# arkworks-rs/pcd

Hardware: AMD Instinct MI355X
Metric: msm_mscalar_mul_per_s (higher is better)
Workload: dtype u32 (11 x 28-bit unsaturated Montgomery limbs, v_mad_u64_u32 with 64-bit column accumulators); 1 GPU; MNT4-298 G1 variable-base MSM, n=1048576 pairs per GPU (2^20 per GPU), proving-key bases and scalars resident in HBM, scalar distribution uniform; curve=MNT4-298, group=G1, log_n=20, window_bits=20, windows=15

## Files before the change

pcd_amd/csrc/capi_internal.h:

```cpp
#pragma once
#include <string.h>

#include <algorithm>
#include <new>

#include "common.h"

namespace pcd {

const int kFieldLimbs[4] = {5, 5, 12, 12};
const int kCurveFq[4] = {0, 1, 2, 3};
const int kCurveFr[4] = {1, 0, 3, 2};
const int kCurveG2Deg[4] = {2, 3, 2, 3};

inline bool valid_curve(int c) { return c >= 0 && c < 4; }
inline bool valid_field(int f) { return f >= 0 && f < 4; }
inline bool valid_group(int g) { return g == 1 || g == 2; }

template <class Fn>
int guarded(Fn&& body) {
  try { return body(); }
  catch (const std::bad_alloc&) { return PCDHIP_E_OOM; }
  catch (...) { return PCDHIP_E_HIP; }
}

inline int fail(pcdhip_ctx* ctx, hipError_t e) {
  if (ctx) { try { ctx->last_hip_error = hipGetErrorString(e); } catch (...) {} }
  if (e == hipErrorOutOfMemory) return PCDHIP_E_OOM;
  if (e == hipErrorNoDevice || e == hipErrorInvalidDevice) return PCDHIP_E_NO_DEVICE;
  if (e == hipErrorInvalidValue) return PCDHIP_E_ARG;
  return PCDHIP_E_HIP;
}
#define TRY(x) do { hipError_t e_ = (x); if (e_ != hipSuccess) return fail(ctx, e_); } while (0)
#define BIND() do { hipError_t e_ = hipSetDevice(ctx->device); if (e_ != hipSuccess) return fail(ctx, e_); } while (0)

enum { AUX_FFT_X = 0, AUX_FFT_TMP, AUX_A, AUX_B, AUX_C, AUX_Z, AUX_CSR_RP, AUX_CSR_COL, AUX_CSR_COEF, AUX_SCAL, AUX_OUT,
       AUX_G16, AUX_Z_CANON, AUX_H_CANON, AUX_MISC, AUX_FB_TABLE, AUX_FB_JAC, AUX_FB_OUT };

struct Dom { uint32_t n, m; int a; };

template <class T> struct FieldTag { typedef T type; };
template <class Fn>
void with_host_field(int field_id, Fn&& fn) {
  switch (field_id) {
    case 0: fn(FieldTag<Fp<F298A, false>>()); break;
    case 1: fn(FieldTag<Fp<F298B, false>>()); break;
    case 2: fn(FieldTag<Fp<F753A, false>>()); break;
    default: fn(FieldTag<Fp<F753B, false>>()); break;
  }
}

typedef hipError_t (*G1ScaleFn)(hipStream_t, const uint32_t*, const uint32_t*, uint32_t, uint32_t, uint32_t*);
G1ScaleFn g1_scale_entry(int curve_id);

hipError_t zero_flagged(hipStream_t st, uint32_t* pts_dev, uint8_t* flags_dev, const uint8_t* flags_host, size_t n, size_t point_bytes);
void shard_range(size_t n, size_t g, size_t parts, size_t* lo, size_t* hi);
int bases_upload_single(pcdhip_ctx* ctx, int curve_id, int group_id, const uint64_t* xy, const uint8_t* inf, size_t n, pcdhip_bases** out);
int msm_common(pcdhip_ctx* ctx, const pcdhip_bases* bases, size_t offset, const uint32_t* scalars_dev, size_t n, uint64_t* out_xyz,
               bool out_on_device = false);
int ensure_side_streams(pcdhip_ctx* ctx);
int drop_side_streams(pcdhip_ctx* ctx, bool partial);
bool pipe_pending(const pcdhip_ctx* ctx);
void drain_peers(pcdhip_ctx* ctx);

int msm_short_common(pcdhip_ctx* ctx, const pcdhip_bases* bases, size_t offset, const uint32_t* scalars_dev, size_t n, uint64_t* out_xyz);
int msm_short_async(pcdhip_ctx* ctx, const pcdhip_bases* bases, size_t offset, const uint32_t* scalars_dev, size_t n, uint32_t* out_dev);
int msm_short_host(pcdhip_ctx* ctx, const pcdhip_bases* bases, size_t offset, const uint64_t* scalars, size_t n, uint64_t* out_xyz);
int msm_short_batch_async(pcdhip_ctx* ctx, const pcdhip_bases* bases, const MsmShortBatchIn* items, size_t k, uint32_t* out_dev,
                          size_t out_stride_words, const uint32_t** err_dev = nullptr, uint32_t* launches = nullptr);

int pick_domain(int field_id, size_t min_size, Dom* d);
int get_tables(pcdhip_ctx* ctx, int field_id, int log_n, const FftTables** out);
int get_mixed_tables(pcdhip_ctx* ctx, int field_id, const Dom& d, const FftTables** out);
int domain_transform(pcdhip_ctx* ctx, int field_id, const Dom& d, uint32_t* v, uint32_t* tmp, int inverse, int coset, float* pass_ms,
                     int* npasses);

size_t csr_bytes(const pcdhip_csr* m, const FieldEntry& fe, size_t off[6]);
int validate_csr(const pcdhip_csr* m, size_t num_cols);
int upload_csr_to(pcdhip_ctx* ctx, const pcdhip_csr* m, const FieldEntry& fe, size_t num_cols, char* d, DevCsr* out);
int upload_csr(pcdhip_ctx* ctx, int slot, const pcdhip_csr* m, const FieldEntry& fe, size_t num_cols, DevCsr* out);
int upload_three(pcdhip_ctx* ctx, const pcdhip_csr* A, const pcdhip_csr* B, const pcdhip_csr* C, const FieldEntry& fe, size_t num_vars,
                 DevCsr out[3]);
int witness_chain_dev(pcdhip_ctx* ctx, int field_id, const DevCsr& mat, int k, const uint32_t* z_dev, size_t num_inputs, const Dom& d, int slot,
                      bool transforms = true);
int witness_finish_dev(pcdhip_ctx* ctx, int field_id, const Dom& d, const uint32_t* b_at = nullptr, const uint32_t* c_at = nullptr);
int witness_map_dev(pcdhip_ctx* ctx, int field_id, const DevCsr mats[3], const uint32_t* z_dev, size_t num_inputs, Dom* dom_out,
                    hipEvent_t after_spmv = nullptr);

struct HostCsrT {
  std::vector<uint64_t> rp;
  std::vector<uint32_t> col;
  std::vector<uint64_t> coeff;
  pcdhip_csr view;
};
int transpose_csr(const pcdhip_csr* m, size_t cols, size_t limbs, HostCsrT* t, const uint32_t* perm = nullptr, size_t rows_out = 0);

void negate_point(int curve_id, int group_id, uint64_t* xy);
void scalar_lincomb(int fr, const uint64_t* const* a, const uint64_t* const* b, size_t n, uint64_t* out);

}

struct pcdhip_pvk {
  int curve_id = 0;
  size_t num_inputs = 0;
  std::vector<uint64_t> alpha, beta, neg_gamma, neg_delta, gamma_abc, alpha_beta , gt_one;
  std::vector<uint8_t> gamma_abc_inf;
  pcdhip_bases* abc = nullptr;
  uint32_t* abc_dev = nullptr;
  size_t abc_tables_off = 0;
};
constexpr size_t PVK_TABLE_INPUTS = 256;
```

pcd_amd/csrc/capi_msm.hip:

```cpp
#include <mutex>

#include "capi_internal.h"

using namespace pcd;

namespace {
__global__ void __launch_bounds__(256) zero_flagged_kernel(uint32_t* __restrict__ pts, const uint8_t* __restrict__ flags, size_t n_words,
                                                            uint32_t words_per_point) {
  const size_t i = (size_t)blockIdx.x * blockDim.x + threadIdx.x;
  if (i < n_words && flags[i / words_per_point]) pts[i] = 0;
}

int lane_reserve_of(const pcdhip_ctx* ctx) {
  int r = ctx->lane_reserve;
  if (r < 0) { const char* e = getenv("PCDHIP_LANE_RESERVE"); r = e ? atoi(e) : 8; }
  return r < 0 ? 0 : r;
}
hipStream_t masked_lane_of(int device, int cus, int reserve, hipError_t* err) {
  static std::mutex mu;
  static std::map<std::pair<int, int>, hipStream_t> pool;
  std::lock_guard<std::mutex> lock(mu);
  auto it = pool.find({device, reserve});
  if (it != pool.end()) { *err = hipSuccess; return it->second; }
  std::vector<uint32_t> mask((cus + 31) / 32, 0u);
  for (int i = 0; i < cus - reserve; i++) mask[i / 32] |= 1u << (i % 32);
  hipStream_t s = nullptr;
  *err = hipExtStreamCreateWithCUMask(&s, (uint32_t)mask.size(), mask.data());
  if (*err == hipSuccess) pool[{device, reserve}] = s;
  return s;
}
int make_side_streams(pcdhip_ctx* ctx) {
  int least = 0, greatest = 0;
  TRY(hipDeviceGetStreamPriorityRange(&least, &greatest));
  const bool lane_mode = ctx->g16_schedule == 2;
  int cus = 0;
  if (hipDeviceGetAttribute(&cus, hipDeviceAttributeMultiprocessorCount, ctx->device) != hipSuccess || cus <= 0) cus = 256;
  const int normal = (least + greatest) / 2;
  for (int k = 0; k < 6; k++) {
    int prio = lane_mode ? (k < 2 ? greatest : k < 4 ? normal : least) : (k < 2 ? greatest : k == 2 ? normal : least);
    static const char* side_prio = getenv("PCDHIP_SIDE_PRIO");
    if (side_prio && !strcmp(side_prio, "low")) prio = least;
    if (side_prio && !strcmp(side_prio, "mid")) prio = k < 3 ? normal : least;
    TRY(hipStreamCreateWithPriority(&ctx->g16_streams[k], hipStreamNonBlocking, prio));
    TRY(hipEventCreate(&ctx->g16_begin[k]));
    TRY(hipEventCreate(&ctx->g16_end[k]));
  }
  if (lane_mode) {
    int reserve = lane_reserve_of(ctx);
    if (reserve >= cus) reserve = 0;
    if (reserve > 0) {
      hipError_t e = hipSuccess;
      ctx->lane.stream = masked_lane_of(ctx->device, cus, reserve, &e);
      TRY(e);
    } else {
      TRY(hipStreamCreateWithPriority(&ctx->lane_stream, hipStreamNonBlocking, least));
      ctx->lane.stream = ctx->lane_stream;
    }
    ctx->lane.cus = cus - reserve;
  }
  TRY(hipEventCreateWithFlags(&ctx->g16_ready, hipEventDisableTiming));
  return PCDHIP_OK;
}
}

namespace pcd {
int msm_coarse_tile_knob() {
  static const int knob = [] {
    const char* e = getenv("PCDHIP_COARSE_TILE");
    if (!e || *e < '0' || *e > '9') return -1;
    const int v = atoi(e);
    return v == 0 || (v >= (int)MSM_STAGE_TILE_MIN && v <= (int)MSM_STAGE_TILE_MAX) ? v : -1;
  }();
  return knob;
}

int msm_bin_stage_knob() {
  static const int knob = [] {
    const char* e = getenv("PCDHIP_BIN_STAGE");
    return e && e[0] == '0' && e[1] == 0 ? 0 : -1;
  }();
  return knob;
}

hipError_t zero_flagged(hipStream_t st, uint32_t* pts_dev, uint8_t* flags_dev, const uint8_t* flags_host, size_t n, size_t point_bytes) {
  if (!flags_host || !n) return hipSuccess;
  hipError_t e = hipMemcpyAsync(flags_dev, flags_host, n, hipMemcpyHostToDevice, st);
  if (e != hipSuccess) return e;
  const size_t nw = n * (point_bytes / 4);
  hipLaunchKernelGGL(zero_flagged_kernel, dim3((unsigned)((nw + 255) / 256)), dim3(256), 0, st, pts_dev, flags_dev, nw, (uint32_t)(point_bytes / 4));
  return hipGetLastError();
}

void shard_range(size_t n, size_t g, size_t parts, size_t* lo, size_t* hi) {
  const size_t base = n / parts, rem = n % parts;
  *lo = g * base + std::min(g, rem);
  *hi = *lo + base + (g < rem ? 1 : 0);
}
int bases_upload_single(pcdhip_ctx* ctx, int curve_id, int group_id, const uint64_t* xy, const uint8_t* inf, size_t n, pcdhip_bases** out) {
  BIND();
  const GroupEntry& ge = group_entry(curve_id, group_id);
  const size_t abi_b = (size_t)ge.point_abi_words * 4, int_b = (size_t)ge.base_stride_words * 4;
  pcdhip_bases* b = new (std::nothrow) pcdhip_bases();
  if (!b) return PCDHIP_E_OOM;
  b->curve_id = curve_id; b->group_id = group_id; b->n = n; b->dptr = nullptr; b->c = 0; b->groups = 1;
  if (ctx->precompute != 0 && n >= 64) {
    const bool full = ctx->precompute < 0;
    const int c = ctx->msm_c ? ctx->msm_c : std::max(6, msm_pick_window(n, ge.scalar_bits, full ? 1 : 0) + ctx->msm_c_bias);
    const int W = msm_num_windows(ge.scalar_bits, c);
    b->c = c;
    b->groups = full ? W : std::min(W, ctx->precompute);
  }
  hipError_t e = hipErrorOutOfMemory;
  while (true) {
    const size_t want = std::max<size_t>(n, 1) * int_b * b->groups;
    e = (ctx->precompute_budget && want > ctx->precompute_budget && b->groups > 1) ? hipErrorOutOfMemory : hipMalloc(&b->dptr, want);
    if (e == hipSuccess || b->groups == 1) break;
    (void)hipGetLastError();
    b->groups = (b->groups + 1) / 2;
  }
  if (e != hipSuccess) { (void)hipGetLastError(); delete b; return fail(ctx, e); }
  if (b->groups == 1) b->c = 0;
  e = ctx->aux_ws.ensure(AUX_MISC, std::max<size_t>(n, 1) * (abi_b + 1) + 64);
  char* stage = (char*)ctx->aux_ws.buf[AUX_MISC];
  if (e == hipSuccess) e = hipMemcpyAsync(stage, xy, n * abi_b, hipMemcpyHostToDevice, ctx->stream);
  if (e == hipSuccess) e = zero_flagged(ctx->stream, (uint32_t*)stage, (uint8_t*)stage + n * abi_b, inf, n, abi_b);
  if (e == hipSuccess) e = ge.points_in(ctx->stream, (const uint32_t*)stage, (uint32_t)n, b->dptr);
  if (e == hipSuccess && b->groups > 1) {
    const int W = msm_num_windows(ge.scalar_bits, b->c);
    const int Wg = (W + b->groups - 1) / b->groups;
    e = ge.precompute(ctx->stream, b->dptr, (uint32_t)n, b->groups, b->c * Wg);
  }
  if (e == hipSuccess && inf) {
    std::vector<uint32_t> bits((n + 31) / 32 + 1, 0u);
    bool any = false;
    for (size_t i = 0; i < n; i++) if (inf[i]) { bits[i >> 5] |= 1u << (i & 31); any = true; }
    if (any) {
      e = hipMalloc((void**)&b->inf_bits, bits.size() * 4);
      if (e == hipSuccess) e = hipMemcpyAsync(b->inf_bits, bits.data(), bits.size() * 4, hipMemcpyHostToDevice, ctx->stream);
      if (e == hipSuccess) e = hipStreamSynchronize(ctx->stream);
    }
  }
  if (e == hipSuccess) e = hipStreamSynchronize(ctx->stream);
  if (e != hipSuccess) { (void)hipFree(b->dptr); (void)hipFree(b->inf_bits); delete b; return fail(ctx, e); }
  *out = b;
  return PCDHIP_OK;
}

int msm_common(pcdhip_ctx* ctx, const pcdhip_bases* bases, size_t offset, const uint32_t* scalars_dev, size_t n,
               uint64_t* out_xyz, bool out_on_device) {
  const GroupEntry& ge = group_entry(bases->curve_id, bases->group_id);
  const size_t jac_b = (size_t)ge.point_words / 2 * 3 * 4, jac_abi_b = (size_t)ge.point_abi_words / 2 * 3 * 4;
  TRY(ctx->msm_ws.ensure(WS_OUT, jac_b + jac_abi_b + 64));
  uint32_t* out_dev = (uint32_t*)ctx->msm_ws.buf[WS_OUT];
  uint32_t* out_abi = out_dev + jac_b / 4;
  TRY(ge.msm(ctx->msm_ws, ctx->stream, bases->view(offset), scalars_dev, (uint32_t)n, out_dev, ctx->msm_c, ctx->msm_chunk,
             ctx->msm_sort, ctx->msm_profile ? &ctx->msm_tm : nullptr, nullptr, MSM_SHARE_NONE));
  if (out_on_device) { TRY(ge.jac_out(ctx->stream, out_dev, 1, (uint32_t*)out_xyz)); return PCDHIP_OK; }
  TRY(ge.jac_out(ctx->stream, out_dev, 1, out_abi));
  TRY(hipMemcpyAsync(out_xyz, out_abi, jac_abi_b, hipMemcpyDeviceToHost, ctx->stream));
  uint32_t too_wide = 0;
  if (ctx->msm_ws.last_err_dev) TRY(hipMemcpyAsync(&too_wide, ctx->msm_ws.last_err_dev, 4, hipMemcpyDeviceToHost, ctx->stream));
  TRY(hipStreamSynchronize(ctx->stream));
  return too_wide ? PCDHIP_E_ARG : PCDHIP_OK;
}

int ensure_side_streams(pcdhip_ctx* ctx) {
  if (ctx->g16_ready) return PCDHIP_OK;
  const int rc = make_side_streams(ctx);
  if (rc) (void)drop_side_streams(ctx, true);
  return rc;
}
int drop_side_streams(pcdhip_ctx* ctx, bool partial) {
  if (!ctx->g16_ready && !partial) return PCDHIP_OK;
  BIND();
  if (!partial) TRY(hipDeviceSynchronize());
  for (int k = 0; k < 6; k++) {
    if (ctx->g16_streams[k]) { (void)hipStreamDestroy(ctx->g16_streams[k]); ctx->g16_streams[k] = nullptr; }
    if (ctx->g16_begin[k]) { (void)hipEventDestroy(ctx->g16_begin[k]); ctx->g16_begin[k] = nullptr; }
    if (ctx->g16_end[k]) { (void)hipEventDestroy(ctx->g16_end[k]); ctx->g16_end[k] = nullptr; }
  }
  if (ctx->lane_stream) { (void)hipStreamDestroy(ctx->lane_stream); ctx->lane_stream = nullptr; }
  ctx->lane = MsmLane();
  if (ctx->g16_ready) (void)hipEventDestroy(ctx->g16_ready);
  ctx->g16_ready = nullptr;
  return PCDHIP_OK;
}
bool pipe_pending(const pcdhip_ctx* ctx) {
  for (int k = 0; k < pcdhip_ctx::PIPE_SLOTS; k++) if (ctx->pipe_busy[k]) return true;
  return false;
}

void drain_peers(pcdhip_ctx* ctx) {
  for (pcdhip_ctx* C : ctx->peers) { if (hipSetDevice(C->device) == hipSuccess) (void)hipStreamSynchronize(C->stream); }
  (void)hipSetDevice(ctx->device);
  (void)hipStreamSynchronize(ctx->stream);
}
}

namespace {
int msm_submit_common(pcdhip_ctx* ctx, const pcdhip_bases* bases, size_t offset, const pcdhip_buf* scalars, size_t scalar_offset, size_t n,
                      uint64_t* out_xyz_device, size_t out_slot_stride, int* ticket) {
  if (!ctx || !bases || !scalars || !ticket || !bases->shards.empty()) return PCDHIP_E_ARG;
  if (offset + n > bases->n || scalar_offset + n > scalars->n || n >= (1ull << 31)) return PCDHIP_E_ARG;
  if (scalars->field_id != kCurveFr[bases->curve_id]) return PCDHIP_E_ARG;
  BIND();
  int rc = ensure_side_streams(ctx);
  if (rc) return rc;
  int slot = -1;
  for (int t = 0; t < pcdhip_ctx::PIPE_SLOTS; t++) {
    const int k = (ctx->pipe_next + t) % pcdhip_ctx::PIPE_SLOTS;
    if (!ctx->pipe_busy[k]) { slot = k; break; }
  }
  if (slot < 0) return PCDHIP_E_ARG;
  ctx->pipe_next = (slot + 1) % pcdhip_ctx::PIPE_SLOTS;
  if (!ctx->pipe_host) TRY(hipHostMalloc((void**)&ctx->pipe_host, pcdhip_ctx::PIPE_SLOTS * pcdhip_ctx::PIPE_HOST_WORDS * 8, hipHostMallocDefault));
  if (!ctx->pipe_done[slot]) TRY(hipEventCreateWithFlags(&ctx->pipe_done[slot], hipEventDisableTiming));
  bool prev_bad = false;
  if (ctx->pipe_partial[slot]) {
    TRY(hipEventSynchronize(ctx->pipe_done[slot]));
    ctx->pipe_partial[slot] = false;
    prev_bad = (uint32_t)ctx->pipe_host[(size_t)slot * pcdhip_ctx::PIPE_HOST_WORDS + pcdhip_ctx::PIPE_HOST_WORDS - 1] != 0;
  }
  const GroupEntry& ge = group_entry(bases->curve_id, bases->group_id);
  const size_t jac_b = (size_t)ge.point_words / 2 * 3 * 4, jac_abi_b = (size_t)ge.point_abi_words / 2 * 3 * 4;
  MsmWorkspace& ws = ctx->g16_ws[2 + slot];
  hipStream_t sk = ctx->g16_streams[2 + slot];
  TRY(ws.ensure(WS_OUT, jac_b + jac_abi_b + 64));
  uint32_t* out_dev = (uint32_t*)ws.buf[WS_OUT];
  uint32_t* out_abi = out_xyz_device ? (uint32_t*)((char*)out_xyz_device + (size_t)slot * out_slot_stride) : out_dev + jac_b / 4;
  TRY(hipEventRecord(ctx->g16_ready, ctx->stream));
  TRY(hipStreamWaitEvent(sk, ctx->g16_ready, 0));
  const size_t sw = (size_t)kFieldLimbs[scalars->field_id] * 2;
  ws.lane = ctx->g16_schedule == 2 && ctx->pipe_lane && ctx->lane.stream ? &ctx->lane : nullptr;
  const hipError_t me = ge.msm(ws, sk, bases->view(offset), scalars->dptr + scalar_offset * sw, (uint32_t)n, out_dev, ctx->msm_c, ctx->msm_chunk, ctx->msm_sort,
                               nullptr, nullptr, MSM_SHARE_NONE);
  ws.lane = nullptr;
  TRY(me);
  TRY(ge.jac_out(sk, out_dev, 1, out_abi));
  uint64_t* host = ctx->pipe_host + (size_t)slot * pcdhip_ctx::PIPE_HOST_WORDS;
  host[pcdhip_ctx::PIPE_HOST_WORDS - 1] = 0;
  if (!out_xyz_device) TRY(hipMemcpyAsync(host, out_abi, jac_abi_b, hipMemcpyDeviceToHost, sk));
  if (ws.last_err_dev) TRY(hipMemcpyAsync(&host[pcdhip_ctx::PIPE_HOST_WORDS - 1], ws.last_err_dev, 4, hipMemcpyDeviceToHost, sk));
  TRY(hipEventRecord(ctx->pipe_done[slot], sk));
  ctx->pipe_busy[slot] = true;
  ctx->pipe_out_bytes[slot] = out_xyz_device ? 0 : jac_abi_b;
  *ticket = slot;
  return prev_bad ? PCDHIP_E_PREV_TICKET : PCDHIP_OK;
}

int msm_sharded_impl(pcdhip_ctx* ctx, const pcdhip_bases* bases, size_t offset, const uint64_t* scalars, size_t n, uint64_t* out_xyz,
                     uint32_t* too_wide) {
  const size_t G = bases->shards.size();
  const GroupEntry& ge = group_entry(bases->curve_id, bases->group_id);
  const size_t jb = (size_t)ge.point_abi_words / 2 * 3 * 4, ji = (size_t)ge.point_words / 2 * 3 * 4;
  const size_t sl = (size_t)kFieldLimbs[kCurveFr[bases->curve_id]];
  BIND();
  TRY(ctx->aux_ws.ensure(AUX_MISC, (G + 1) * jb + 64 * ji + 64));
  uint32_t* d = (uint32_t*)ctx->aux_ws.buf[AUX_MISC];
  uint32_t* gather = d + jb / 4;
  uint32_t* scratch = d + (G + 1) * jb / 4;
  for (size_t g = 0; g < G; g++) {
    const size_t lo = std::max(offset, bases->shard_lo[g]), hi = std::min(offset + n, bases->shard_lo[g + 1]);
    pcdhip_ctx* C = ctx->peers[g];
    if (hi <= lo) {
      TRY(hipSetDevice(ctx->device));
      TRY(hipMemsetAsync((char*)gather + g * jb, 0, jb, ctx->stream));
      continue;
    }
    const pcdhip_bases* sh = bases->shards[g];
    const size_t ng = hi - lo;
    C->msm_sort = ctx->msm_sort;
    {
      pcdhip_ctx* ctx = C;
      BIND();
      const size_t sbytes = ng * sl * 8;
      TRY(C->msm_ws.ensure(WS_SCAL, std::max<size_t>(sbytes, 8)));
      TRY(C->msm_ws.ensure(WS_OUT, ji + jb + 64));
      TRY(hipMemcpyAsync(C->msm_ws.buf[WS_SCAL], scalars + (lo - offset) * sl, sbytes, hipMemcpyHostToDevice, C->stream));
      uint32_t* out_dev = (uint32_t*)C->msm_ws.buf[WS_OUT];
      uint32_t* out_abi = out_dev + ji / 4;
      TRY(ge.msm(C->msm_ws, C->stream, sh->view(lo - bases->shard_lo[g]), (const uint32_t*)C->msm_ws.buf[WS_SCAL], (uint32_t)ng, out_dev, C->msm_c,
                 C->msm_chunk, C->msm_sort, nullptr, nullptr, MSM_SHARE_NONE));
      TRY(ge.jac_out(C->stream, out_dev, 1, out_abi));
      if (C->msm_ws.last_err_dev) TRY(hipMemcpyAsync(&too_wide[g], C->msm_ws.last_err_dev, 4, hipMemcpyDeviceToHost, C->stream));
    }
    const uint32_t* out_abi = (const uint32_t*)C->msm_ws.buf[WS_OUT] + ji / 4;
    TRY(hipSetDevice(C->device));
    TRY(hipMemcpyPeerAsync((char*)gather + g * jb, ctx->device, out_abi, C->device, jb, C->stream));
    if (C != ctx) {
      if (!C->xstream_ev) TRY(hipEventCreateWithFlags(&C->xstream_ev, hipEventDisableTiming));
      TRY(hipEventRecord(C->xstream_ev, C->stream));
      TRY(hipSetDevice(ctx->device));
      TRY(hipStreamWaitEvent(ctx->stream, C->xstream_ev, 0));
    }
  }
  BIND();
  TRY(ge.points_sum(ctx->stream, gather, (uint32_t)G, scratch, d));
  TRY(hipMemcpyAsync(out_xyz, d, jb, hipMemcpyDeviceToHost, ctx->stream));
  for (size_t g = 1; g < G; g++) { TRY(hipSetDevice(ctx->peers[g]->device)); TRY(hipStreamSynchronize(ctx->peers[g]->stream)); }
  BIND();
  TRY(hipStreamSynchronize(ctx->stream));
  for (size_t g = 0; g < G; g++) if (too_wide[g]) return PCDHIP_E_ARG;
  return PCDHIP_OK;
}
int msm_sharded(pcdhip_ctx* ctx, const pcdhip_bases* bases, size_t offset, const uint64_t* scalars, size_t n, uint64_t* out_xyz) {
  if (ctx->peers.size() != bases->shards.size() || ctx->peers.size() > 64) return PCDHIP_E_ARG;
  uint32_t too_wide[64] = {0};
  const int rc = msm_sharded_impl(ctx, bases, offset, scalars, n, out_xyz, too_wide);
  if (rc) drain_peers(ctx);
  return rc;
}

int points_sum_common(pcdhip_ctx* ctx, int curve_id, int group_id, const uint64_t* xyz, size_t n, uint64_t* out_xyz, bool in_on_device) {
  if (!ctx || !valid_curve(curve_id) || !valid_group(group_id) || (!xyz && n) || !out_xyz || (n >> 24)) return PCDHIP_E_ARG;
  BIND();
  const GroupEntry& ge = group_entry(curve_id, group_id);
  const size_t jb = (size_t)ge.point_abi_words / 2 * 3 * 4, ji = (size_t)ge.point_words / 2 * 3 * 4;
  TRY(ctx->aux_ws.ensure(AUX_MISC, (n + 1) * jb + 64 * ji + 64));
  uint32_t* d = (uint32_t*)ctx->aux_ws.buf[AUX_MISC];
  uint32_t* scratch = d + (n + 1) * jb / 4;
  const uint32_t* in = (const uint32_t*)xyz;
  if (!in_on_device) {
    TRY(hipMemcpyAsync(d + jb / 4, xyz, n * jb, hipMemcpyHostToDevice, ctx->stream));
    in = d + jb / 4;
  }
  TRY(ge.points_sum(ctx->stream, in, (uint32_t)n, scratch, d));
  TRY(hipMemcpyAsync(out_xyz, d, jb, hipMemcpyDeviceToHost, ctx->stream));
  TRY(hipStreamSynchronize(ctx->stream));
  return PCDHIP_OK;
}
}

extern "C" {

int pcdhip_bases_upload(pcdhip_ctx* ctx, int curve_id, int group_id, const uint64_t* xy, const uint8_t* inf, size_t n,
                        pcdhip_bases** out) {
  if (!ctx || !out || !valid_curve(curve_id) || !valid_group(group_id) || (!xy && n) || n >= (1ull << 31)) return PCDHIP_E_ARG;
  if (ctx->peers.size() <= 1) return bases_upload_single(ctx, curve_id, group_id, xy, inf, n, out);
  *out = nullptr;
  return guarded([&]() -> int {
    pcdhip_bases* b = new pcdhip_bases();
    b->curve_id = curve_id; b->group_id = group_id; b->n = n; b->dptr = nullptr; b->c = 0; b->groups = 1;
    const size_t G = ctx->peers.size(), pl = (size_t)pcdhip_point_limbs(curve_id, group_id);
    b->shard_lo.resize(G + 1);
    for (size_t g = 0; g < G; g++) {
      size_t lo, hi;
      shard_range(n, g, G, &lo, &hi);
      b->shard_lo[g] = lo; b->shard_lo[g + 1] = hi;
      pcdhip_ctx* C = ctx->peers[g];
      C->precompute = ctx->precompute; C->precompute_budget = ctx->precompute_budget; C->msm_c = ctx->msm_c;
      pcdhip_bases* sh = nullptr;
      int rc = bases_upload_single(C, curve_id, group_id, xy + lo * pl, inf ? inf + lo : nullptr, hi - lo, &sh);
      if (rc) { pcdhip_bases_free(ctx, b); return rc; }
      b->shards.push_back(sh);
    }
    *out = b;
    return PCDHIP_OK;
  });
}
int pcdhip_set_precompute(pcdhip_ctx* ctx, int mode) {
  if (!ctx || mode < -1 || mode == 1) return PCDHIP_E_ARG;
  ctx->precompute = mode;
  return PCDHIP_OK;
}
int pcdhip_set_precompute_budget(pcdhip_ctx* ctx, size_t bytes_per_vector) {
  if (!ctx) return PCDHIP_E_ARG;
  ctx->precompute_budget = bytes_per_vector;
  return PCDHIP_OK;
}
int pcdhip_get_precompute_budget(pcdhip_ctx* ctx, size_t* bytes_per_vector) {
  if (!ctx || !bytes_per_vector) return PCDHIP_E_ARG;
  *bytes_per_vector = ctx->precompute_budget;
  return PCDHIP_OK;
}
void pcdhip_bases_free(pcdhip_ctx* ctx, pcdhip_bases* bases) {
  if (!bases) return;
  for (size_t g = 0; g < bases->shards.size(); g++)
    pcdhip_bases_free(ctx && g < ctx->peers.size() ? ctx->peers[g] : ctx, bases->shards[g]);
  bases->shards.clear();
  if (ctx) (void)hipSetDevice(ctx->device);
  (void)hipFree(bases->dptr);
  (void)hipFree(bases->inf_bits);
  delete bases;
}
int pcdhip_bases_info(const pcdhip_bases* bases, size_t n, int* window_bits, int* windows, int* copies) {
  if (!bases || !window_bits || !windows || !copies) return PCDHIP_E_ARG;
  if (!bases->shards.empty()) return pcdhip_bases_info(bases->shards[0], 0, window_bits, windows, copies);
  const GroupEntry& ge = group_entry(bases->curve_id, bases->group_id);
  const int c = bases->groups > 1 ? bases->c : msm_pick_window(n ? n : bases->n, ge.scalar_bits, 0);
  *window_bits = c;
  *windows = msm_num_windows(ge.scalar_bits, c);
  *copies = bases->groups;
  return PCDHIP_OK;
}
int pcdhip_msm_config(pcdhip_ctx* ctx, int window_bits, int chunk) {
  if (!ctx || window_bits < 0 || window_bits > 24 || chunk < 0) return PCDHIP_E_ARG;
  ctx->msm_c = window_bits;
  ctx->msm_chunk = (uint32_t)chunk;
  return PCDHIP_OK;
}
int pcdhip_msm_set_sort(pcdhip_ctx* ctx, int mode) {
  if (!ctx || mode < 0 || mode > 4) return PCDHIP_E_ARG;
  ctx->msm_sort = (ctx->msm_sort & ~15) | mode;
  return PCDHIP_OK;
}
int pcdhip_msm_set_bin_stage(pcdhip_ctx* ctx, int cap) {
  if (!ctx || cap < -1 || cap > (int)MSM_BIN_STAGE_CAP) return PCDHIP_E_ARG;
  const std::vector<pcdhip_ctx*> one{ctx};
  for (pcdhip_ctx* c : ctx->peers.empty() ? one : ctx->peers) {
    c->msm_ws.bin_stage = cap;
    for (pcd::MsmWorkspace& w : c->g16_ws) w.bin_stage = cap;
  }
  return PCDHIP_OK;
}
int pcdhip_msm_set_accumulate(pcdhip_ctx* ctx, int mode, int chunk, int min_pairs) {
  if (!ctx || mode < 0 || mode > 2 || chunk < 0 || chunk > 1024 || (chunk && chunk < 2) || min_pairs < 0 || min_pairs > 255) return PCDHIP_E_ARG;
  ctx->msm_sort = (ctx->msm_sort & 15) | (mode << 4) | (chunk << 8) | (min_pairs << 20);
  return PCDHIP_OK;
}
int pcdhip_msm_profile(pcdhip_ctx* ctx, int on) {
  if (!ctx) return PCDHIP_E_ARG;
  ctx->msm_profile = on != 0;
  return PCDHIP_OK;
}
int pcdhip_msm_last_plan(pcdhip_ctx* ctx, uint32_t out[2]) {
  if (!ctx || !out) return PCDHIP_E_ARG;
  out[0] = ctx->msm_tm.entries; out[1] = ctx->msm_tm.chunk;
  return PCDHIP_OK;
}
int pcdhip_msm_last_timings(pcdhip_ctx* ctx, float out_ms[8]) {
  if (!ctx || !out_ms) return PCDHIP_E_ARG;
  const MsmTimings& t = ctx->msm_tm;
  float v[8] = {t.digits, t.scan, t.scatter, t.accumulate, t.fixup, t.tail, t.horner, t.total};
  memcpy(out_ms, v, sizeof v);
  return PCDHIP_OK;
}

int pcdhip_msm_ticket_status(pcdhip_ctx* ctx, int slot) {
  if (!ctx || slot < 0 || slot >= pcdhip_ctx::PIPE_SLOTS || ctx->pipe_busy[slot] || !ctx->pipe_partial[slot]) return PCDHIP_E_ARG;
  BIND();
  TRY(hipEventSynchronize(ctx->pipe_done[slot]));
  ctx->pipe_partial[slot] = false;
  return (uint32_t)ctx->pipe_host[(size_t)slot * pcdhip_ctx::PIPE_HOST_WORDS + pcdhip_ctx::PIPE_HOST_WORDS - 1] ? PCDHIP_E_PREV_TICKET : PCDHIP_OK;
}
int pcdhip_msm_submit(pcdhip_ctx* ctx, const pcdhip_bases* bases, size_t offset, const pcdhip_buf* scalars, size_t scalar_offset, size_t n,
                      int* ticket) {
  const int rc = msm_submit_common(ctx, bases, offset, scalars, scalar_offset, n, nullptr, 0, ticket);
  return rc == PCDHIP_E_PREV_TICKET ? PCDHIP_OK : rc;
}
int pcdhip_msm_submit_partial(pcdhip_ctx* ctx, const pcdhip_bases* bases, size_t offset, const pcdhip_buf* scalars, size_t scalar_offset, size_t n,
                              uint64_t* out_xyz_device_slots, size_t slot_stride_bytes, int* ticket) {
  if (!out_xyz_device_slots || (slot_stride_bytes & 7)) return PCDHIP_E_ARG;
  return msm_submit_common(ctx, bases, offset, scalars, scalar_offset, n, out_xyz_device_slots, slot_stride_bytes, ticket);
}
int pcdhip_msm_ticket_wait(pcdhip_ctx* ctx, int ticket, void* other_stream) {
  if (!ctx || ticket < 0 || ticket >= pcdhip_ctx::PIPE_SLOTS || !ctx->pipe_busy[ticket]) return PCDHIP_E_ARG;
  BIND();
  TRY(hipStreamWaitEvent((hipStream_t)other_stream, ctx->pipe_done[ticket], 0));
  ctx->pipe_busy[ticket] = false;
  ctx->pipe_partial[ticket] = true;
  return PCDHIP_OK;
}
int pcdhip_msm_collect(pcdhip_ctx* ctx, int ticket, uint64_t* out_xyz) {
  if (!ctx || ticket < 0 || ticket >= pcdhip_ctx::PIPE_SLOTS || !ctx->pipe_busy[ticket] || !out_xyz) return PCDHIP_E_ARG;
  BIND();
  ctx->pipe_busy[ticket] = false;
  TRY(hipEventSynchronize(ctx->pipe_done[ticket]));
  const uint64_t* host = ctx->pipe_host + (size_t)ticket * pcdhip_ctx::PIPE_HOST_WORDS;
  memcpy(out_xyz, host, ctx->pipe_out_bytes[ticket]);
  return (uint32_t)host[pcdhip_ctx::PIPE_HOST_WORDS - 1] ? PCDHIP_E_ARG : PCDHIP_OK;
}

int pcdhip_msm_dev(pcdhip_ctx* ctx, const pcdhip_bases* bases, size_t offset, const pcdhip_buf* scalars, size_t scalar_offset,
                   size_t n, uint64_t* out_xyz) {
  if (!ctx || !bases || !scalars || !out_xyz) return PCDHIP_E_ARG;
  if (!bases->shards.empty()) return PCDHIP_E_ARG;
  if (offset + n > bases->n || scalar_offset + n > scalars->n || n >= (1ull << 31)) return PCDHIP_E_ARG;
  if (scalars->field_id != kCurveFr[bases->curve_id]) return PCDHIP_E_ARG;
  BIND();
  const size_t sw = (size_t)kFieldLimbs[scalars->field_id] * 2;
  return msm_common(ctx, bases, offset, scalars->dptr + scalar_offset * sw, n, out_xyz);
}

int pcdhip_msm_dev_partial(pcdhip_ctx* ctx, const pcdhip_bases* bases, size_t offset, const pcdhip_buf* scalars, size_t scalar_offset,
                           size_t n, uint64_t* out_xyz_device) {
  if (!ctx || !bases || !scalars || !out_xyz_device || !bases->shards.empty()) return PCDHIP_E_ARG;
  if (offset + n > bases->n || scalar_offset + n > scalars->n || n >= (1ull << 31)) return PCDHIP_E_ARG;
  if (scalars->field_id != kCurveFr[bases->curve_id]) return PCDHIP_E_ARG;
  BIND();
  const size_t sw = (size_t)kFieldLimbs[scalars->field_id] * 2;
  return msm_common(ctx, bases, offset, scalars->dptr + scalar_offset * sw, n, out_xyz_device, true);
}

int pcdhip_msm(pcdhip_ctx* ctx, const pcdhip_bases* bases, size_t offset, const uint64_t* scalars, size_t n, uint64_t* out_xyz) {
  if (!ctx || !bases || (!scalars && n) || !out_xyz) return PCDHIP_E_ARG;
  if (offset + n > bases->n || n >= (1ull << 31)) return PCDHIP_E_ARG;
  if (!bases->shards.empty()) return msm_sharded(ctx, bases, offset, scalars, n, out_xyz);
  BIND();
  const size_t sbytes = n * kFieldLimbs[kCurveFr[bases->curve_id]] * 8;
  TRY(ctx->msm_ws.ensure(WS_SCAL, std::max<size_t>(sbytes, 8)));
  TRY(hipMemcpyAsync(ctx->msm_ws.buf[WS_SCAL], scalars, sbytes, hipMemcpyHostToDevice, ctx->stream));
  return msm_common(ctx, bases, offset, (const uint32_t*)ctx->msm_ws.buf[WS_SCAL], n, out_xyz);
}

int pcdhip_points_sum(pcdhip_ctx* ctx, int curve_id, int group_id, const uint64_t* xyz, size_t n, uint64_t* out_xyz) {
  return points_sum_common(ctx, curve_id, group_id, xyz, n, out_xyz, false);
}
int pcdhip_points_sum_dev(pcdhip_ctx* ctx, int curve_id, int group_id, const uint64_t* xyz_device, size_t n, uint64_t* out_xyz) {
  return points_sum_common(ctx, curve_id, group_id, xyz_device, n, out_xyz, true);
}

int pcdhip_to_affine(pcdhip_ctx* ctx, int curve_id, int group_id, const uint64_t* xyz, size_t n, uint64_t* out_xy, uint8_t* out_inf) {
  if (!ctx || !valid_curve(curve_id) || !valid_group(group_id) || (!xyz && n) || !out_xy) return PCDHIP_E_ARG;
  BIND();
  const GroupEntry& ge = group_entry(curve_id, group_id);
  const size_t ab = (size_t)ge.point_abi_words * 4, jb = ab / 2 * 3;
  TRY(ctx->aux_ws.ensure(AUX_MISC, n * (jb + ab) + 64));
  uint32_t* dj = (uint32_t*)ctx->aux_ws.buf[AUX_MISC];
  uint32_t* da = dj + n * jb / 4;
  TRY(hipMemcpyAsync(dj, xyz, n * jb, hipMemcpyHostToDevice, ctx->stream));
  TRY(ge.to_affine(ctx->stream, dj, (uint32_t)n, da));
  TRY(hipMemcpyAsync(out_xy, da, n * ab, hipMemcpyDeviceToHost, ctx->stream));
  TRY(hipStreamSynchronize(ctx->stream));
  if (out_inf) {
    for (size_t i = 0; i < n; i++) {
      const uint64_t* p = out_xy + i * (ab / 8);
      uint64_t o = 0;
      for (size_t k = 0; k < ab / 8; k++) o |= p[k];
      out_inf[i] = (o == 0) ? 1 : 0;
    }
  }
  return PCDHIP_OK;
}

}
```

pcd_amd/csrc/msm.hip.h:

```cpp
#pragma once
#include <cstdlib>
#include <math.h>

#include <algorithm>
#include <atomic>
#include <type_traits>
#include <vector>

#include "ec.hip.h"

namespace pcd {

template <int K>
struct EventSet {
  hipEvent_t e[K] = {};
  bool live = false;
  hipError_t create() {
    for (int i = 0; i < K; i++) { hipError_t r = hipEventCreate(&e[i]); if (r != hipSuccess) return r; }
    live = true;
    return hipSuccess;
  }
  hipEvent_t operator[](int i) const { return e[i]; }
  ~EventSet() { for (int i = 0; i < K; i++) if (e[i]) (void)hipEventDestroy(e[i]); }
};

struct MsmPlan {
  uint32_t n = 0;
  int c = 0;
  int W = 0;
  uint32_t nkeys = 0;
  uint32_t chunk = 0;
};

PCD_HD constexpr int msm_num_windows(int scalar_bits, int c) { return (scalar_bits + c) / c; }

inline int msm_pick_window(size_t n, int scalar_bits, int full_precompute) {
  double best = 1e300;
  int bc = 8;
  for (int c = 6; c <= 22; c++) {
    int W = msm_num_windows(scalar_bits, c);
    int Wg = full_precompute ? 1 : W;
    double cost = (double)W * (double)n * 11.0 + (double)Wg * (double)(1u << c) * 16.0 * 1.3;
    int top = scalar_bits + 1 - (W - 1) * c;
    cost += (double)n / (double)(1u << (top > 20 ? 20 : top)) * 1400.0;
    if (cost < best) { best = cost; bc = c; }
  }
  return bc;
}

constexpr uint32_t MSM_NEG = 0x80000000u;
PCD_DEV uint32_t msm_signed(uint32_t raw, int c, uint32_t& carry, uint32_t& neg) {
  uint32_t d = raw + carry;
  const bool n = d > (1u << (c - 1));
  carry = n ? 1u : 0u;
  neg = n ? MSM_NEG : 0u;
  return n ? (1u << c) - d : d;
}
template <int NS>
PCD_DEV bool msm_scalar_too_wide(const uint32_t* s, int bits) {
  uint32_t o = 0;
#pragma unroll
  for (int k = 0; k < NS; k++) {
    if (32 * k >= bits) o |= s[k];
    else if (32 * (k + 1) > bits) o |= s[k] >> (bits - 32 * k);
  }
  return o != 0;
}
PCD_DEV bool msm_base_is_inf(const uint32_t* __restrict__ inf_bits, uint32_t idx) { return inf_bits && ((inf_bits[idx >> 5] >> (idx & 31u)) & 1u); }
template <int NS>
PCD_DEV uint32_t msm_digit(const uint32_t* s, int w, int c) {
  int bit = w * c;
  int word = bit >> 5, off = bit & 31;
  uint64_t x = s[word];
  if (word + 1 < NS) x |= (uint64_t)s[word + 1] << 32;
  return (uint32_t)(x >> off) & ((1u << c) - 1u);
}

enum { MODE_HIST = 0, MODE_SCATTER = 1, MODE_BIN = 2 };
template <int NS, int MODE>
__global__ void __launch_bounds__(256) msm_digits_kernel(const uint32_t* __restrict__ scalars, uint32_t n, int c, int W, int Wg,
                                                         uint32_t n_total, uint32_t base_offset, uint32_t nkeys,
                                                         uint32_t* __restrict__ cnt, const uint32_t* __restrict__ off,
                                                         uint32_t* __restrict__ sorted_idx, uint32_t* __restrict__ slots, uint32_t cap,
                                                         uint32_t* __restrict__ ones_idx, uint32_t* __restrict__ flag, int skip_ones,
                                                         int scalar_bits, uint32_t* __restrict__ err, const uint32_t* __restrict__ inf_bits) {
  if (MODE == MODE_SCATTER && flag && *flag == 0) return;
  uint32_t i = blockIdx.x * blockDim.x + threadIdx.x;
  bool live = i < n && !msm_base_is_inf(inf_bits, base_offset + i);
  uint32_t s[NS];
  bool is_one = false;
  if (live || (i < n && MODE != MODE_SCATTER && err)) {
    uint32_t hi = 0;
#pragma unroll
    for (int k = 0; k < NS; k++) { s[k] = scalars[(size_t)i * NS + k]; if (k) hi |= s[k]; }
    is_one = live && (hi == 0 && s[0] == 1);
    if (MODE != MODE_SCATTER && err && msm_scalar_too_wide<NS>(s, scalar_bits)) *err = 1u;
  }
  unsigned long long m = __ballot(live && is_one);
  if (m && !skip_ones) {
    int lane = threadIdx.x & 63;
    int leader = __ffsll((long long)m) - 1;
    uint32_t base = 0;
    if (lane == leader) base = atomicAdd(&cnt[nkeys], (uint32_t)__popcll(m));
    if (MODE != MODE_HIST) {
      base = __shfl(base, leader, 64);
      if (live && is_one) {
        uint32_t rank = (uint32_t)__popcll(m & ((1ull << lane) - 1ull));
        if (MODE == MODE_BIN) ones_idx[base + rank] = base_offset + i;
        else sorted_idx[off[nkeys] + base + rank] = base_offset + i;
      }
    }
  }
  if (!live || is_one) return;
  int g = 0, j = 0;
  uint32_t carry = 0, neg;
  for (int w = 0; w < W; w++) {
    uint32_t d = msm_signed(msm_digit<NS>(s, w, c), c, carry, neg);
    if (d != 0) {
      uint32_t key = ((uint32_t)j << c) | d;
      uint32_t pos = atomicAdd(&cnt[key], 1u);
      uint32_t idx = ((uint32_t)g * n_total + base_offset + i) | neg;
      if (MODE == MODE_SCATTER) sorted_idx[off[key] + pos] = idx;
      if (MODE == MODE_BIN) {
        if (pos < cap) slots[(size_t)key * cap + pos] = idx;
        else *flag = 1u;
      }
    }
    if (++j == Wg) { j = 0; g++; }
  }
}

#ifndef PCD_SORT_UNROLL
#define PCD_SORT_UNROLL 4
#endif
constexpr int MSM_SORT_UNROLL = PCD_SORT_UNROLL;
constexpr int MSM_BIN_SHIFT = 9;
#ifndef PCD_MSM_TILE
#define PCD_MSM_TILE 2048
#endif
constexpr int MSM_TILE = PCD_MSM_TILE;
constexpr uint32_t MSM_MAX_BINS = 8192;

template <int NS, bool WRITE>
__global__ void __launch_bounds__(256) msm_coarse_kernel(const uint32_t* __restrict__ scalars, uint32_t n, int c, int W, int Wg,
                                                         uint32_t n_total, uint32_t base_offset, uint32_t nbins,
                                                         uint32_t* __restrict__ gbin ,
                                                         uint64_t* __restrict__ entries, uint32_t* __restrict__ ones_count,
                                                         uint32_t* __restrict__ ones_idx, int scalar_bits, uint32_t* __restrict__ err,
                                                         const uint32_t* __restrict__ inf_bits) {
  extern __shared__ uint32_t lbin[];
  __shared__ uint32_t s_ones[WRITE ? 1 : MSM_TILE];
  __shared__ uint32_t s_nones, s_ones_base;
  for (uint32_t b = threadIdx.x; b < nbins; b += blockDim.x) lbin[b] = 0;
  if (threadIdx.x == 0) s_nones = 0;
  __syncthreads();
  const uint32_t tile0 = blockIdx.x * MSM_TILE;
  for (uint32_t k = threadIdx.x; k < MSM_TILE; k += blockDim.x) {
    uint32_t i = tile0 + k;
    bool live = i < n && !msm_base_is_inf(inf_bits, base_offset + i);
    uint32_t s[NS];
    bool is_one = false;
    if (live || (i < n && !WRITE)) {
      uint32_t hi = 0;
#pragma unroll
      for (int q = 0; q < NS; q++) { s[q] = scalars[(size_t)i * NS + q]; if (q) hi |= s[q]; }
      is_one = live && (hi == 0 && s[0] == 1);
      if (!WRITE && msm_scalar_too_wide<NS>(s, scalar_bits)) *err = 1u;
    }
    if (!WRITE) {
      unsigned long long m = __ballot(live && is_one);
      if (m) {
        int lane = threadIdx.x & 63;
        int leader = __ffsll((long long)m) - 1;
        uint32_t base = 0;
        if (lane == leader) base = atomicAdd(&s_nones, (uint32_t)__popcll(m));
        base = __shfl(base, leader, 64);
        if (live && is_one) s_ones[base + (uint32_t)__popcll(m & ((1ull << lane) - 1ull))] = base_offset + i;
      }
    }
    if (!live || is_one) continue;
    int j = 0;
    uint32_t carry = 0, neg;
    for (int w = 0; w < W; w++) {
      uint32_t d = msm_signed(msm_digit<NS>(s, w, c), c, carry, neg);
      if (d != 0) atomicAdd(&lbin[((((uint32_t)j << c) | d)) >> MSM_BIN_SHIFT], 1u);
      if (++j == Wg) j = 0;
    }
  }
  __syncthreads();
  for (uint32_t b = threadIdx.x; b < nbins; b += blockDim.x) {
    uint32_t cnt = lbin[b];
    if (cnt) {
      uint32_t base = atomicAdd(&gbin[b], cnt);
      if (WRITE) lbin[b] = base;
    }
  }
  if (!WRITE) {
    if (threadIdx.x == 0) s_ones_base = s_nones ? atomicAdd(ones_count, s_nones) : 0u;
    __syncthreads();
    for (uint32_t k = threadIdx.x; k < s_nones; k += blockDim.x) ones_idx[s_ones_base + k] = s_ones[k];
    return;
  }
  __syncthreads();
  for (uint32_t k = threadIdx.x; k < MSM_TILE; k += blockDim.x) {
    uint32_t i = tile0 + k;
    if (i >= n || msm_base_is_inf(inf_bits, base_offset + i)) continue;
    uint32_t s[NS];
    uint32_t hi = 0;
#pragma unroll
    for (int q = 0; q < NS; q++) { s[q] = scalars[(size_t)i * NS + q]; if (q) hi |= s[q]; }
    if (hi == 0 && s[0] <= 1) continue;
    int g = 0, j = 0;
    uint32_t carry = 0, neg;
    for (int w = 0; w < W; w++) {
      uint32_t d = msm_signed(msm_digit<NS>(s, w, c), c, carry, neg);
      if (d != 0) {
        uint32_t key = ((uint32_t)j << c) | d;
        uint32_t pos = atomicAdd(&lbin[key >> MSM_BIN_SHIFT], 1u);
        entries[pos] = ((uint64_t)key << 32) | (uint64_t)(((uint32_t)g * n_total + base_offset + i) | neg);
      }
      if (++j == Wg) { j = 0; g++; }
    }
  }
}

constexpr int MSM_STAGE_G_BITS = 6, MSM_STAGE_IDX_BITS = 11;
constexpr uint32_t MSM_STAGE_TILE_MAX = 1u << MSM_STAGE_IDX_BITS, MSM_STAGE_TILE_MIN = 256;
constexpr int MSM_STAGE_W_MAX = 1 << MSM_STAGE_G_BITS;
constexpr int MSM_STAGE_SIGN_AT = MSM_BIN_SHIFT, MSM_STAGE_G_AT = MSM_BIN_SHIFT + 1, MSM_STAGE_IDX_AT = MSM_STAGE_G_AT + MSM_STAGE_G_BITS;
static_assert(MSM_STAGE_IDX_AT + MSM_STAGE_IDX_BITS <= 32, "staged word: low key bits, sign, group and tile index in 32 bits");
constexpr size_t MSM_STAGE_LDS_BUDGET = 152u * 1024u;
constexpr uint32_t MSM_STAGE_MIN_RUN = 8;
PCD_HD constexpr size_t msm_stage_lds_bytes(uint32_t tile, int W, uint32_t nbins) { return 4 * ((size_t)tile * (size_t)W + 3 * (size_t)nbins + 4); }
PCD_HD constexpr uint32_t msm_stage_tile(int W, uint32_t nbins) {
  if (W < 1 || W > MSM_STAGE_W_MAX || nbins < 1) return 0;
  for (uint32_t t = MSM_STAGE_TILE_MAX; t >= MSM_STAGE_TILE_MIN; t >>= 1)
    if (msm_stage_lds_bytes(t, W, nbins) <= MSM_STAGE_LDS_BUDGET) return (uint64_t)t * (uint32_t)W >= (uint64_t)MSM_STAGE_MIN_RUN * nbins ? t : 0;
  return 0;
}
int msm_coarse_tile_knob();

constexpr int msm_stage_block(int TILE) { return TILE < 1024 ? TILE : 1024; }
template <int NS, int TILE>
__global__ void __launch_bounds__(msm_stage_block(TILE)) msm_coarse_staged_kernel(const uint32_t* __restrict__ scalars, uint32_t n, int c, int W, int Wg,
                                                                                  uint32_t n_total, uint32_t base_offset, uint32_t nbins,
                                                                                  uint32_t* __restrict__ gbin ,
                                                                                  uint64_t* __restrict__ entries, const uint32_t* __restrict__ inf_bits) {
  constexpr int BLOCK = msm_stage_block(TILE), K = TILE / BLOCK, NW = BLOCK / 64;
  static_assert(TILE >= (int)MSM_STAGE_TILE_MIN && TILE <= (int)MSM_STAGE_TILE_MAX && TILE % BLOCK == 0, "tile");
  extern __shared__ uint32_t lds[];
  uint32_t* cur = lds;
  uint32_t* loff = cur + nbins;
  uint32_t* rdelta = loff + nbins + 1;
  uint32_t* buf = rdelta + nbins;
  __shared__ uint32_t s_wsum[NW];
  const uint32_t t = threadIdx.x, tile0 = blockIdx.x * TILE;
  for (uint32_t b = t; b < nbins; b += BLOCK) cur[b] = 0;
  uint32_t s[K][NS];
  bool live[K];
#pragma unroll
  for (int kk = 0; kk < K; kk++) {
    const uint32_t i = tile0 + t + kk * BLOCK;
    live[kk] = i < n && !msm_base_is_inf(inf_bits, base_offset + i);
    uint32_t hi = 0;
#pragma unroll
    for (int q = 0; q < NS; q++) { s[kk][q] = live[kk] ? scalars[(size_t)i * NS + q] : 0u; if (q) hi |= s[kk][q]; }
    if (hi == 0 && s[kk][0] <= 1) live[kk] = false;
  }
  __syncthreads();
#pragma unroll
  for (int kk = 0; kk < K; kk++) {
    if (!live[kk]) continue;
    int j = 0;
    uint32_t carry = 0, neg;
    for (int w = 0; w < W; w++) {
      uint32_t d = msm_signed(msm_digit<NS>(s[kk], w, c), c, carry, neg);
      if (d != 0) atomicAdd(&cur[((((uint32_t)j << c) | d)) >> MSM_BIN_SHIFT], 1u);
      if (++j == Wg) j = 0;
    }
  }
  __syncthreads();
  const uint32_t per = (nbins + BLOCK - 1) / BLOCK;
  const uint32_t blo = min(nbins, t * per), bhi = min(nbins, blo + per);
  uint32_t acc = 0;
  for (uint32_t b = blo; b < bhi; b++) acc += cur[b];
  const uint32_t lane = t & 63, wv = t >> 6;
  uint32_t incl = acc;
  for (int d = 1; d < 64; d <<= 1) { uint32_t o = __shfl_up(incl, d, 64); if ((int)lane >= d) incl += o; }
  if (lane == 63) s_wsum[wv] = incl;
  __syncthreads();
  uint32_t run = incl - acc;
  for (uint32_t q = 0; q < wv; q++) run += s_wsum[q];
  for (uint32_t b = blo; b < bhi; b++) {
    const uint32_t cnt = cur[b];
    loff[b] = run;
    cur[b] = run;
    if (cnt) rdelta[b] = atomicAdd(&gbin[b], cnt) - run;
    run += cnt;
  }
  if (t == BLOCK - 1) loff[nbins] = run;
  __syncthreads();
#pragma unroll
  for (int kk = 0; kk < K; kk++) {
    if (!live[kk]) continue;
    int g = 0, j = 0;
    uint32_t carry = 0, neg;
    for (int w = 0; w < W; w++) {
      uint32_t d = msm_signed(msm_digit<NS>(s[kk], w, c), c, carry, neg);
      if (d != 0) {
        const uint32_t key = ((uint32_t)j << c) | d;
        const uint32_t q = atomicAdd(&cur[key >> MSM_BIN_SHIFT], 1u);
        buf[q] = (key & ((1u << MSM_BIN_SHIFT) - 1u)) | (neg ? 1u << MSM_STAGE_SIGN_AT : 0u) | ((uint32_t)g << MSM_STAGE_G_AT) |
                 ((t + kk * BLOCK) << MSM_STAGE_IDX_AT);
      }
      if (++j == Wg) { j = 0; g++; }
    }
  }
  __syncthreads();
  const uint32_t total = loff[nbins];
  for (uint32_t q = t; q < total; q += BLOCK) {
    const uint32_t word = buf[q];
    uint32_t lo = 0, hi = nbins;
    while (hi - lo > 1) {
      const uint32_t mid = (lo + hi) >> 1;
      if (loff[mid] <= q) lo = mid; else hi = mid;
    }
    const uint32_t key = (lo << MSM_BIN_SHIFT) | (word & ((1u << MSM_BIN_SHIFT) - 1u));
    const uint32_t g = (word >> MSM_STAGE_G_AT) & ((1u << MSM_STAGE_G_BITS) - 1u);
    const uint32_t neg = (word >> MSM_STAGE_SIGN_AT) & 1u ? MSM_NEG : 0u;
    const uint32_t idx = (g * n_total + base_offset + tile0 + (word >> MSM_STAGE_IDX_AT)) | neg;
    entries[rdelta[lo] + q] = ((uint64_t)key << 32) | (uint64_t)idx;
  }
}
template <int NS, int TILE>
hipError_t msm_coarse_staged_launch(hipStream_t st, uint32_t tiles, size_t lds, const uint32_t* scalars, uint32_t n, int c, int W, int Wg,
                                    uint32_t n_total, uint32_t base_offset, uint32_t nbins, uint32_t* gbin, uint64_t* entries,
                                    const uint32_t* inf_bits) {
  static std::atomic<uint64_t> allowed{0};
  int dev = 0;
  hipError_t e = hipGetDevice(&dev);
  if (e != hipSuccess) return e;
  const uint64_t bit = 1ull << (dev & 63);
  if (!(allowed.load(std::memory_order_relaxed) & bit)) {
    e = hipFuncSetAttribute(reinterpret_cast<const void*>(&msm_coarse_staged_kernel<NS, TILE>), hipFuncAttributeMaxDynamicSharedMemorySize,
                            (int)MSM_STAGE_LDS_BUDGET);
    if (e != hipSuccess) return e;
    allowed.fetch_or(bit, std::memory_order_relaxed);
  }
  hipLaunchKernelGGL((msm_coarse_staged_kernel<NS, TILE>), dim3(tiles), dim3(msm_stage_block(TILE)), lds, st, scalars, n, c, W, Wg, n_total,
                     base_offset, nbins, gbin, entries, inf_bits);
  return hipSuccess;
}

static __global__ void __launch_bounds__(1024) msm_bin_scan_kernel(const uint32_t* __restrict__ bin_cnt, uint32_t nbins,
                                                                   uint32_t* __restrict__ bin_base, uint32_t* __restrict__ cursor,
                                                                   const uint32_t* __restrict__ ones_count, uint32_t* __restrict__ off,
                                                                   uint32_t nkeys) {
  __shared__ uint32_t part[1024];
  const uint32_t per = (nbins + 1023) / 1024;
  const uint32_t lo = threadIdx.x * per, hi = min(nbins, lo + per);
  uint32_t acc = 0;
  for (uint32_t b = lo; b < hi; b++) acc += bin_cnt[b];
  part[threadIdx.x] = acc;
  __syncthreads();
  for (int s = 1; s < 1024; s <<= 1) {
    uint32_t t = ((int)threadIdx.x >= s) ? part[threadIdx.x - s] : 0;
    __syncthreads();
    part[threadIdx.x] += t;
    __syncthreads();
  }
  uint32_t run = part[threadIdx.x] - acc;
  for (uint32_t b = lo; b < hi; b++) { bin_base[b] = run; cursor[b] = run; run += bin_cnt[b]; }
  if (threadIdx.x == 1023) {
    uint32_t M = part[1023];
    bin_base[nbins] = M;
    off[nkeys] = M;
    off[nkeys + 1] = M + *ones_count;
  }
}

template <int BLOCK>
__device__ __forceinline__ void msm_bin_scan_counters(uint32_t* hist, uint32_t* wsum, uint32_t lo, uint32_t hbase, uint32_t* __restrict__ off_b) {
  constexpr int KB = 1 << MSM_BIN_SHIFT, PER = KB / BLOCK;
  static_assert(PER >= 1 && PER * BLOCK == KB && BLOCK % 64 == 0, "counters per lane");
  const uint32_t t = threadIdx.x, lane = t & 63, wv = t >> 6;
  uint32_t c[PER], sum = 0;
#pragma unroll
  for (int k = 0; k < PER; k++) { c[k] = hist[PER * t + k]; sum += c[k]; }
  uint32_t incl = sum;
  for (int d = 1; d < 64; d <<= 1) { uint32_t o = __shfl_up(incl, d, 64); if ((int)lane >= d) incl += o; }
  if (lane == 63) wsum[wv] = incl;
  __syncthreads();
  uint32_t ex = incl - sum;
  for (uint32_t q = 0; q < wv; q++) ex += wsum[q];
#pragma unroll
  for (int k = 0; k < PER; k++) {
    hist[PER * t + k] = hbase + ex;
    off_b[PER * t + k] = lo + ex;
    ex += c[k];
  }
  __syncthreads();
}
template <int BLOCK>
__device__ __forceinline__ void msm_bin_sort_two_read(const uint64_t* __restrict__ entries, uint32_t lo, uint32_t hi, uint32_t* __restrict__ sorted_idx,
                                                      uint32_t* __restrict__ off_b, uint32_t* hist, uint32_t* wsum) {
  constexpr uint32_t KB = 1u << MSM_BIN_SHIFT;
  for (uint32_t k = threadIdx.x; k < KB; k += BLOCK) hist[k] = 0;
  __syncthreads();
  for (uint32_t p0 = lo + threadIdx.x; p0 < hi; p0 += MSM_SORT_UNROLL * BLOCK) {
    uint32_t kk[MSM_SORT_UNROLL];
#pragma unroll
    for (int u = 0; u < MSM_SORT_UNROLL; u++) { uint32_t p = p0 + u * BLOCK; kk[u] = p < hi ? (uint32_t)(entries[p] >> 32) & (KB - 1) : KB; }
#pragma unroll
    for (int u = 0; u < MSM_SORT_UNROLL; u++) if (kk[u] < KB) atomicAdd(&hist[kk[u]], 1u);
  }
  __syncthreads();
  msm_bin_scan_counters<BLOCK>(hist, wsum, lo, lo, off_b);
  for (uint32_t p0 = lo + threadIdx.x; p0 < hi; p0 += MSM_SORT_UNROLL * BLOCK) {
    uint64_t e[MSM_SORT_UNROLL];
    uint32_t pos[MSM_SORT_UNROLL];
#pragma unroll
    for (int u = 0; u < MSM_SORT_UNROLL; u++) { uint32_t p = p0 + u * BLOCK; e[u] = p < hi ? entries[p] : ~0ull; }
#pragma unroll
    for (int u = 0; u < MSM_SORT_UNROLL; u++) if (e[u] != ~0ull) pos[u] = atomicAdd(&hist[(uint32_t)(e[u] >> 32) & (KB - 1)], 1u);
#pragma unroll
    for (int u = 0; u < MSM_SORT_UNROLL; u++) if (e[u] != ~0ull) sorted_idx[pos[u]] = (uint32_t)e[u];
  }
}
static __global__ void __launch_bounds__(256) msm_bin_sort_kernel(const uint64_t* __restrict__ entries, const uint32_t* __restrict__ bin_base,
                                                                  uint32_t* __restrict__ sorted_idx, uint32_t* __restrict__ off) {
  constexpr uint32_t KB = 1u << MSM_BIN_SHIFT;
  __shared__ uint32_t hist[KB];
  __shared__ uint32_t wsum[4];
  const uint32_t b = blockIdx.x;
  msm_bin_sort_two_read<256>(entries, bin_base[b], bin_base[b + 1], sorted_idx, off + (size_t)b * KB, hist, wsum);
}

constexpr int MSM_BIN_STAGE_BLOCK = 512, MSM_BIN_STAGE_PER = 36;
constexpr uint32_t MSM_BIN_STAGE_CAP = MSM_BIN_STAGE_BLOCK * MSM_BIN_STAGE_PER;
PCD_HD constexpr size_t msm_bin_stage_lds_bytes() { return 4 * ((size_t)MSM_BIN_STAGE_CAP + 4 + (1u << MSM_BIN_SHIFT) + MSM_BIN_STAGE_BLOCK / 64); }
static_assert(2 * msm_bin_stage_lds_bytes() <= 160u * 1024u && msm_bin_stage_lds_bytes() <= 78u * 1024u, "two workgroups per CU");
int msm_bin_stage_knob();

static __global__ void __launch_bounds__(MSM_BIN_STAGE_BLOCK, 4) msm_bin_sort_staged_kernel(const uint64_t* __restrict__ entries,
                                                                                             const uint32_t* __restrict__ bin_base,
                                                                                             uint32_t* __restrict__ sorted_idx ,
                                                                                             uint32_t* __restrict__ off, uint32_t cap) {
  constexpr uint32_t KB = 1u << MSM_BIN_SHIFT;
  constexpr int BLOCK = MSM_BIN_STAGE_BLOCK, PER = MSM_BIN_STAGE_PER;
  static_assert(MSM_BIN_STAGE_CAP % 4 == 0 && MSM_BIN_STAGE_CAP < (1u << (32 - MSM_BIN_SHIFT)), "16-byte lines; the rank beside the key");
  extern __shared__ __attribute__((aligned(16))) uint32_t bin_lds[];
  uint32_t* buf = bin_lds;
  uint32_t* hist = buf + MSM_BIN_STAGE_CAP + 4;
  uint32_t* wsum = hist + KB;
  const uint32_t b = blockIdx.x, t = threadIdx.x, lo = bin_base[b], hi = bin_base[b + 1], m = hi - lo;
  uint32_t* off_b = off + (size_t)b * KB;
  if (m > min(cap, MSM_BIN_STAGE_CAP)) { msm_bin_sort_two_read<BLOCK>(entries, lo, hi, sorted_idx, off_b, hist, wsum); return; }
  for (uint32_t k = t; k < KB; k += BLOCK) hist[k] = 0;
  __syncthreads();
  uint64_t e[PER];
#pragma unroll
  for (int u = 0; u < PER; u++) { const uint32_t p = lo + t + u * BLOCK; e[u] = p < hi ? entries[p] : 0ull; }
  uint32_t idx[PER], kr[PER];
#pragma unroll
  for (int u = 0; u < PER; u++) {
    const uint32_t k = (uint32_t)(e[u] >> 32) & (KB - 1);
    idx[u] = (uint32_t)e[u];
    kr[u] = ~0u;
    if (lo + t + u * BLOCK < hi) kr[u] = k | (atomicAdd(&hist[k], 1u) << MSM_BIN_SHIFT);
  }
  __syncthreads();
  const uint32_t sh = lo & 3u;
  msm_bin_scan_counters<BLOCK>(hist, wsum, lo, sh, off_b);
#pragma unroll
  for (int u = 0; u < PER; u++)
    if (kr[u] != ~0u) buf[hist[kr[u] & (KB - 1)] + (kr[u] >> MSM_BIN_SHIFT)] = idx[u];
  __syncthreads();
  const uint32_t end = sh + m;
  uint32_t* dst = sorted_idx + (lo - sh);
  for (uint32_t q = 4 * t; q < end; q += 4 * BLOCK) {
    if (q >= sh && q + 4 <= end) {
      *reinterpret_cast<uint4*>(dst + q) = *reinterpret_cast<const uint4*>(buf + q);
    } else {
#pragma unroll
      for (uint32_t w = 0; w < 4; w++) if (q + w >= sh && q + w < end) dst[q + w] = buf[q + w];
    }
  }
}
static hipError_t msm_bin_sort_launch(hipStream_t st, uint32_t nbins, uint32_t cap, const uint64_t* entries, const uint32_t* bin_base,
                                      uint32_t* sorted_idx, uint32_t* off) {
  if (!cap) {
    hipLaunchKernelGGL(msm_bin_sort_kernel, dim3(nbins), dim3(256), 0, st, entries, bin_base, sorted_idx, off);
    return hipSuccess;
  }
  static std::atomic<uint64_t> allowed{0};
  int dev = 0;
  hipError_t e = hipGetDevice(&dev);
  if (e != hipSuccess) return e;
  const uint64_t bit = 1ull << (dev & 63);
  if (!(allowed.load(std::memory_order_relaxed) & bit)) {
    e = hipFuncSetAttribute(reinterpret_cast<const void*>(&msm_bin_sort_staged_kernel), hipFuncAttributeMaxDynamicSharedMemorySize,
                            (int)msm_bin_stage_lds_bytes());
    if (e != hipSuccess) return e;
    allowed.fetch_or(bit, std::memory_order_relaxed);
  }
  hipLaunchKernelGGL(msm_bin_sort_staged_kernel, dim3(nbins), dim3(MSM_BIN_STAGE_BLOCK), msm_bin_stage_lds_bytes(), st, entries, bin_base,
                     sorted_idx, off, std::min(cap, MSM_BIN_STAGE_CAP));
  return hipSuccess;
}

static __global__ void __launch_bounds__(1024) scan_block_sums(const uint32_t* __restrict__ in, uint32_t n, uint32_t per_block,
                                                         uint32_t* __restrict__ block_sums) {
  __shared__ uint32_t sh[1024];
  uint32_t b = blockIdx.x, lo = b * per_block, hi = min(n, lo + per_block);
  uint32_t acc = 0;
  for (uint32_t i = lo + threadIdx.x; i < hi; i += blockDim.x) acc += in[i];
  sh[threadIdx.x] = acc;
  __syncthreads();
  for (int s = 512; s > 0; s >>= 1) { if ((int)threadIdx.x < s) sh[threadIdx.x] += sh[threadIdx.x + s]; __syncthreads(); }
  if (threadIdx.x == 0) block_sums[b] = sh[0];
}
static __global__ void __launch_bounds__(1024) scan_apply(const uint32_t* __restrict__ in, uint32_t n, uint32_t per_block,
                                                    const uint32_t* __restrict__ block_sums, uint32_t nblocks,
                                                    uint32_t* __restrict__ out ) {
  __shared__ uint32_t sh[1024];
  __shared__ uint32_t carry;
  uint32_t b = blockIdx.x, lo = b * per_block, hi = min(n, lo + per_block);
  if (threadIdx.x == 0) { uint32_t a = 0; for (uint32_t k = 0; k < b; k++) a += block_sums[k]; carry = a; }
  __syncthreads();
  for (uint32_t base = lo; base < hi; base += 1024) {
    uint32_t i = base + threadIdx.x;
    uint32_t v = (i < hi) ? in[i] : 0;
    sh[threadIdx.x] = v;
    __syncthreads();
    for (int s = 1; s < 1024; s <<= 1) {
      uint32_t t = ((int)threadIdx.x >= s) ? sh[threadIdx.x - s] : 0;
      __syncthreads();
      sh[threadIdx.x] += t;
      __syncthreads();
    }
    if (i < hi) out[i] = carry + sh[threadIdx.x] - v;
    __syncthreads();
    if (threadIdx.x == 0) carry += sh[1023];
    __syncthreads();
  }
  if (b == nblocks - 1 && threadIdx.x == 0) out[n] = carry;
}

PCD_HD uint64_t msm_plan_rounds(uint32_t M, uint32_t lanes, uint32_t hi) {
  const uint64_t per_round = (uint64_t)lanes * hi;
  return ((uint64_t)M + per_round - 1) / per_round;
}
PCD_HD uint32_t msm_plan_chunk(uint32_t M, uint32_t lanes, uint32_t lo, uint32_t hi) {
  const uint64_t rounds = msm_plan_rounds(M, lanes, hi);
  const uint32_t chunk = rounds ? (uint32_t)(((uint64_t)M + (uint64_t)lanes * rounds - 1) / ((uint64_t)lanes * rounds)) : lo;
  return chunk < lo ? lo : chunk > hi ? hi : chunk;
}
constexpr uint32_t MSM_CHUNK_MAX = 128;
#ifndef PCD_CHUNK_HI
#define PCD_CHUNK_HI 56
#endif
constexpr uint32_t MSM_CHUNK_HI = PCD_CHUNK_HI;
PCD_HD uint64_t msm_plan_word(uint32_t lanes, uint32_t lo, uint32_t hi) { return (uint64_t)lanes | ((uint64_t)lo << 20) | ((uint64_t)hi << 28); }
PCD_HD uint32_t msm_chunk_of_plan(uint32_t M, uint64_t plan) {
  return msm_plan_chunk(M, (uint32_t)(plan & 0xFFFFFu), (uint32_t)(plan >> 20) & 255u, (uint32_t)(plan >> 28) & 255u);
}
struct MsmChunkRule {
  const uint32_t* chunk_dev;
  uint64_t plan;
  uint32_t chunk;
  PCD_DEV uint32_t eval(const uint32_t* __restrict__ off, uint32_t nkeys) const {
    return chunk_dev ? *chunk_dev : plan ? msm_chunk_of_plan(off[nkeys], plan) : chunk;
  }
};

PCD_DEV uint32_t msm_find_key(const uint32_t* __restrict__ off, uint32_t nkeys, uint32_t p) {
  uint32_t lo = 0, hi = nkeys;
  while (hi - lo > 1) { uint32_t mid = (lo + hi) >> 1; if (off[mid] <= p) lo = mid; else hi = mid; }
  return lo;
}

struct MsmEntrySource {
  const uint32_t* sorted_idx;
  const uint32_t* slots;
  const uint32_t* ones_idx;
  const uint32_t* flag;
  uint32_t cap, ones_key;
};
struct MsmCursor {
  uint32_t key, key_start, key_end;
  uint32_t next_end;
  PCD_DEV void seek(const uint32_t* __restrict__ off, uint32_t nkeys, uint32_t p) {
    key = msm_find_key(off, nkeys, p);
    key_start = off[key];
    key_end = off[key + 1];
    next_end = key + 2 <= nkeys ? off[key + 2] : key_end;
  }
  PCD_DEV void advance_to(const uint32_t* __restrict__ off, uint32_t nkeys, uint32_t p) {
    for (int step = 0; step < 4 && p >= key_end; step++) {
      key++; key_start = key_end; key_end = next_end;
      next_end = key + 2 <= nkeys ? off[key + 2] : key_end;
    }
    if (p >= key_end) seek(off, nkeys, p);
  }
};
PCD_DEV uint32_t msm_entry(const MsmEntrySource& src, bool compact, const MsmCursor& cur, uint32_t p) {
  if (cur.key == src.ones_key) return compact && !src.ones_idx ? src.sorted_idx[p] : src.ones_idx[p - cur.key_start];
  return compact ? src.sorted_idx[p] : src.slots[(size_t)cur.key * src.cap + (p - cur.key_start)];
}

#ifndef PCD_BASE_ALIGN
#define PCD_BASE_ALIGN 1
#endif
template <class G>
struct MsmBaseStride {
  static constexpr int W = Aff<typename G::F>::WORDS;
  static constexpr int value = (PCD_BASE_ALIGN && W == 22) ? 32 : W;
};

template <class G>
struct MsmUseXyzz {
  typedef typename G::F F;
#ifndef PCD_XYZZ_753
#define PCD_XYZZ_753 0
#endif
  static constexpr bool value = F::Base::INLINE_ARITH || F::DEG == 2 || (PCD_XYZZ_753 && F::Base::N > 11);
};
template <class G, bool XYZZ = MsmUseXyzz<G>::value>
struct MsmRunPlain {
  typedef typename G::F F;
  typename EC<G>::AccX a = EC<G>::x_infinity();
  PCD_DEV void add(const Aff<F>& q) { a = EC<G>::madd_x(a, q); }
  PCD_DEV void flush(uint32_t* dst) {
    a.X.store(dst); a.Y.store(dst + F::WORDS); a.ZZ.store(dst + 2 * F::WORDS); a.ZZZ.store(dst + 3 * F::WORDS);
    a = EC<G>::x_infinity();
  }
};
template <class G>
struct MsmRunPlain<G, false> {
  typedef typename G::F F;
  Jac<F> a = Jac<F>::infinity();
  PCD_DEV void add(const Aff<F>& q) { a = EC<G>::madd(a, q); }
  PCD_DEV void flush(uint32_t* dst) { a.store(dst); a = Jac<F>::infinity(); }
};
template <class G>
struct MsmRunLazy {
  typedef typename G::F F;
  typename EC<G>::AccLz a = EC<G>::lz_infinity();
  PCD_DEV void add(const Aff<F>& q) { a = EC<G>::madd_lz(a, q); }
  PCD_DEV void flush(uint32_t* dst) {
    if (a.inf) { F::zero().store(dst + 2 * F::WORDS); return; }
#pragma unroll
    for (int i = 0; i < F::N; i++) dst[i] = (uint32_t)a.X.v[i];
    a.Y.store(dst + F::WORDS);
    a.ZZ.store(dst + 2 * F::WORDS);
    a.ZZZ.store(dst + 3 * F::WORDS);
    a = EC<G>::lz_infinity();
  }
};
#ifndef PCD_ACC_LDS
#define PCD_ACC_LDS 0
#endif
#if defined(__HIP_DEVICE_COMPILE__) || defined(__HIPCC__)
template <class G>
struct MsmRunLazyLds {
  typedef typename G::F F;
  typedef uint32_t V4 __attribute__((ext_vector_type(4)));
  typedef __attribute__((address_space(3))) V4* LdsV4;
  static constexpr int CH = (F::N + 3) / 4;
  struct Store {
    LdsV4 box;
    bool is_inf;
    PCD_DEV bool& inf() { return is_inf; }
    PCD_DEV F ld(int slot) const {
      F r;
#pragma unroll
      for (int k = 0; k < CH; k++) {
        const V4 w = box[(slot * CH + k) * 64 + threadIdx.x];
        r.v[4 * k] = w.x;
        if (4 * k + 1 < F::N) r.v[4 * k + 1] = w.y;
        if (4 * k + 2 < F::N) r.v[4 * k + 2] = w.z;
        if (4 * k + 3 < F::N) r.v[4 * k + 3] = w.w;
      }
      return r;
    }
    PCD_DEV void st(int slot, const F& a) {
#pragma unroll
      for (int k = 0; k < CH; k++) {
        V4 w;
        w.x = a.v[4 * k];
        w.y = 4 * k + 1 < F::N ? a.v[4 * k + 1] : 0u;
        w.z = 4 * k + 2 < F::N ? a.v[4 * k + 2] : 0u;
        w.w = 4 * k + 3 < F::N ? a.v[4 * k + 3] : 0u;
        box[(slot * CH + k) * 64 + threadIdx.x] = w;
      }
    }
  };
  Store s;
  PCD_DEV MsmRunLazyLds() {
    __shared__ V4 accbox[4 * CH * 64];
    s.box = (LdsV4)accbox;
    s.is_inf = true;
  }
  PCD_DEV void add(const Aff<F>& q) { EC<G>::madd_lz_st(s, q); }
  PCD_DEV void flush(uint32_t* dst) {
    if (s.is_inf) { F::zero().store(dst + 2 * F::WORDS); return; }
    s.ld(0).store(dst); s.ld(1).store(dst + F::WORDS); s.ld(2).store(dst + 2 * F::WORDS); s.ld(3).store(dst + 3 * F::WORDS);
    s.is_inf = true;
  }
};
#endif
template <class G, bool XYZZ = MsmUseXyzz<G>::value>
struct MsmStoredPlain {
  typedef typename G::F F;
  static constexpr int WORDS = EC<G>::ACCX_WORDS;
  PCD_DEV static Jac<F> load(const uint32_t* p) {
    typename EC<G>::AccX a = {F::load(p), F::load(p + F::WORDS), F::load(p + 2 * F::WORDS), F::load(p + 3 * F::WORDS)};
    return EC<G>::x_to_jac(a);
  }
  static constexpr bool SEPARATE = true;
};
template <class G>
struct MsmStoredPlain<G, false> {
  typedef typename G::F F;
  static constexpr int WORDS = Jac<F>::WORDS;
  PCD_DEV static Jac<F> load(const uint32_t* p) { return Jac<F>::load(p); }
  static constexpr bool SEPARATE = false;
};
template <class G, bool LAZY = LazyCapable<typename G::F>::value>
struct MsmStored : MsmStoredPlain<G> {};
template <class G>
struct MsmStored<G, true> {
  typedef typename G::F F;
  static constexpr int WORDS = EC<G>::ACC_WORDS;
  PCD_DEV static Jac<F> load(const uint32_t* p) {
    typename EC<G>::AccLz a;
    a.ZZ = F::load(p + 2 * F::WORDS);
    if (a.ZZ.is_zero()) return Jac<F>::infinity();
    a.inf = false;
#pragma unroll
    for (int i = 0; i < F::N; i++) a.X.v[i] = (int32_t)p[i];
    a.Y = F::load(p + F::WORDS);
    a.ZZZ = F::load(p + 3 * F::WORDS);
    return EC<G>::lz_to_jac(a);
  }
  static constexpr bool SEPARATE = true;
};

template <class G>
struct MsmAccWaves {
  typedef typename AccOf<G>::type::F FA;
#ifndef PCD_ACC_WAVES_SPLIT
#define PCD_ACC_WAVES_SPLIT 2
#endif
#ifndef PCD_ACC_WAVES_G1
#define PCD_ACC_WAVES_G1 2
#endif
#ifndef PCD_ACC_WAVES_MB298
#define PCD_ACC_WAVES_MB298 2
#endif
  static constexpr int value = !FA::Base::INLINE_ARITH ? (FA::Base::N <= 11 ? PCD_ACC_WAVES_MB298 : 1)
                             : FA::DEG == 1 ? PCD_ACC_WAVES_G1 : AccOf<G>::LANES > 1 ? PCD_ACC_WAVES_SPLIT : 1;
};

template <class G, bool COMPACT>
__global__ void __launch_bounds__(64, MsmAccWaves<G>::value) msm_accumulate_kernel(const uint32_t* __restrict__ bases, const MsmEntrySource src,
                                                            const uint32_t* __restrict__ off, uint32_t nkeys,
                                                            uint32_t chunk, uint32_t* __restrict__ buckets,
                                                            uint32_t* __restrict__ piece_first, uint32_t* __restrict__ piece_last,
                                                            uint64_t plan ) {
  if (plan) chunk = msm_chunk_of_plan(off[nkeys], plan);
  typedef typename AccOf<G>::type GA;
  typedef typename GA::F F;
  typedef EC<GA> E;
  constexpr int RW = MsmStored<GA>::WORDS;
  constexpr uint32_t LANES = AccOf<G>::LANES, PER_WAVE = 64 / LANES;
  if (threadIdx.x >= PER_WAVE * LANES) return;
  uint32_t t = blockIdx.x * PER_WAVE + threadIdx.x / LANES;
  const uint32_t M = off[nkeys];
  uint64_t start64 = (uint64_t)t * chunk;
  if (start64 >= M) return;
  uint32_t start = (uint32_t)start64, end = (uint32_t)min((uint64_t)M, start64 + chunk);
  if (!COMPACT && src.flag && *src.flag != 0) return;
  if (COMPACT && src.flag && *src.flag == 0) return;
  MsmCursor cur;
  cur.seek(off, nkeys, start);
  bool open_start = cur.key_start < start;
#if PCD_ACC_LDS
  typename std::conditional<LazyCapable<F>::value, MsmRunLazyLds<GA>, MsmRunPlain<GA>>::type acc;
#else
  typename std::conditional<LazyCapable<F>::value, MsmRunLazy<GA>, MsmRunPlain<GA>>::type acc;
#endif
  constexpr bool PREFETCH = F::Base::INLINE_ARITH;
  const uint32_t ones_start = off[src.ones_key];
  auto point_of = [&](uint32_t e) {
    Aff<F> q = Aff<F>::load(bases + (size_t)(e & ~MSM_NEG) * MsmBaseStride<G>::value);
    const F ny = q.y.neg();
    if (e & MSM_NEG) q.y = ny;
    return q;
  };
  if constexpr (COMPACT) {
    auto entry_at = [&](uint32_t pos) { return (src.ones_idx && pos >= ones_start) ? src.ones_idx[pos - ones_start] : src.sorted_idx[pos]; };
    Aff<F> nxt;
    if (PREFETCH) nxt = point_of(entry_at(start));
    for (uint32_t p = start; p < end; p++) {
      if (p >= cur.key_end) {
        if (open_start) { acc.flush(piece_first + (size_t)t * RW); open_start = false; }
        else acc.flush(buckets + (size_t)cur.key * RW);
        cur.advance_to(off, nkeys, p);
      }
      if (PREFETCH) {
        const Aff<F> pt = nxt;
        if (p + 1 < end) nxt = point_of(entry_at(p + 1));
        acc.add(pt);
      } else {
        acc.add(point_of(entry_at(p)));
      }
    }
  } else {
    MsmCursor nxt_cur = cur;
    Aff<F> nxt;
    if (PREFETCH) nxt = point_of(msm_entry(src, false, cur, start));
    for (uint32_t p = start; p < end; p++) {
      if (p >= cur.key_end) {
        if (open_start) { acc.flush(piece_first + (size_t)t * RW); open_start = false; }
        else acc.flush(buckets + (size_t)cur.key * RW);
        cur.advance_to(off, nkeys, p);
      }
      if (PREFETCH) {
        const Aff<F> pt = nxt;
        if (p + 1 < end) {
          nxt_cur.advance_to(off, nkeys, p + 1);
          nxt = point_of(msm_entry(src, false, nxt_cur, p + 1));
        }
        acc.add(pt);
      } else {
        acc.add(point_of(msm_entry(src, false, cur, p)));
      }
    }
  }
  bool open_end = cur.key_end > end;
  if (open_end) acc.flush(piece_last + (size_t)t * RW);
  else if (open_start) acc.flush(piece_first + (size_t)t * RW);
  else acc.flush(buckets + (size_t)cur.key * RW);
}

constexpr uint32_t MSM_TREE_CHUNK_MAX = 640, MSM_TREE_MIN_PAIRS = 12;
constexpr uint32_t MSM_SCR = 0x40000000u;
template <class G>
struct MsmTreeCapable {
  typedef typename AccOf<G>::type::F F;
  static constexpr bool value = F::DEG == 1 && AccOf<G>::LANES == 1 && F::Base::N > 11;
};
struct MsmTreeBufs {
  uint32_t* list;
  uint32_t* pairs;
  uint32_t* prefix;
  uint32_t* pts;
  uint32_t cap;
  uint32_t phases;
  PCD_HD static size_t list_words(uint32_t cap) { return (size_t)4 * cap * 64; }
  PCD_HD static size_t pair_words(uint32_t cap) { return (size_t)3 * (cap / 2 + 1) * 64; }
  PCD_HD static size_t prefix_words(uint32_t cap, int fw) { return (size_t)((fw + 3) / 4 * 4) * (cap / 2 + 1) * 64; }
  PCD_HD static size_t pts_words(uint32_t cap, int fw) { return (size_t)2 * ((fw + 3) / 4 * 4) * (cap + cap / 4 + 8) * 64; }
};
PCD_DEV uint32_t msm_wave_max(uint32_t v) {
#pragma unroll
  for (int m = 32; m >= 1; m >>= 1) v = max(v, (uint32_t)__shfl_xor((int)v, m, 64));
  return v;
}
enum { MSM_PK_ADD = 0, MSM_PK_TAKE_B = 1, MSM_PK_TAKE_A = 2, MSM_PK_INF = 3, MSM_PK_DBL = 4 };

static __global__ void msm_tree_plan_kernel(const uint32_t* __restrict__ off, uint32_t nkeys, uint32_t lanes, uint32_t cap, uint32_t forced,
                                            uint32_t* __restrict__ chunk_out) {
  if (blockIdx.x || threadIdx.x) return;
  const uint64_t M = off[nkeys];
  const uint64_t rounds = (M + (uint64_t)lanes * cap - 1) / ((uint64_t)lanes * cap);
  uint32_t chunk = rounds ? (uint32_t)((M + lanes * rounds - 1) / (lanes * rounds)) : 32u;
  chunk = min(max(chunk, 32u), cap);
  *chunk_out = forced ? forced : chunk;
}
template <class G>
__global__ void __launch_bounds__(64, 1) msm_pair_tree_kernel(const uint32_t* __restrict__ bases, const MsmEntrySource src,
                                                              const uint32_t* __restrict__ off, uint32_t nkeys, const uint32_t* __restrict__ chunk_dev,
                                                              const MsmTreeBufs tb, uint32_t min_pairs, uint32_t* __restrict__ buckets,
                                                              uint32_t* __restrict__ piece_first, uint32_t* __restrict__ piece_last) {
  typedef typename AccOf<G>::type GA;
  typedef typename GA::F F;
  constexpr int RW = MsmStored<GA>::WORDS, FW = F::WORDS;
  const uint32_t lane = threadIdx.x;
  const uint32_t M = off[nkeys];
  const uint32_t chunk = *chunk_dev;
  const uint32_t nwaves = (uint32_t)((((uint64_t)M + chunk - 1) / chunk + 63) / 64);
  const bool compact = !(src.slots && src.flag && *src.flag == 0);
  const uint32_t ones_start = off[src.ones_key];
  uint32_t* const LS = tb.list + (size_t)blockIdx.x * MsmTreeBufs::list_words(tb.cap) + lane;
  uint32_t* const PR = tb.pairs + (size_t)blockIdx.x * MsmTreeBufs::pair_words(tb.cap) + lane;
  constexpr int ECH = (FW + 3) / 4, EW = 4 * ECH;
  uint32_t* const PX = tb.prefix + (size_t)blockIdx.x * MsmTreeBufs::prefix_words(tb.cap, FW) + lane * 4;
  uint32_t* const PT = tb.pts + (size_t)blockIdx.x * MsmTreeBufs::pts_words(tb.cap, FW) + lane * 4;
  typedef uint32_t V4 __attribute__((ext_vector_type(4)));
  auto fld_ld = [&](const uint32_t* p) { F r;
#pragma unroll
    for (int c = 0; c < ECH; c++) {
      const V4 v = *reinterpret_cast<const V4*>(p + (size_t)c * 256);
      r.v[4 * c] = v.x;
      if (4 * c + 1 < FW) r.v[4 * c + 1] = v.y;
      if (4 * c + 2 < FW) r.v[4 * c + 2] = v.z;
      if (4 * c + 3 < FW) r.v[4 * c + 3] = v.w;
    }
    return r; };
  auto fld_st = [&](uint32_t* p, const F& a) {
#pragma unroll
    for (int c = 0; c < ECH; c++) {
      V4 v;
      v.x = a.v[4 * c];
      v.y = 4 * c + 1 < FW ? a.v[4 * c + 1] : 0u;
      v.z = 4 * c + 2 < FW ? a.v[4 * c + 2] : 0u;
      v.w = 4 * c + 3 < FW ? a.v[4 * c + 3] : 0u;
      *reinterpret_cast<V4*>(p + (size_t)c * 256) = v;
    } };
  auto x_of = [&](uint32_t loc) {
    const bool scr = (loc & MSM_SCR) != 0;
    if (!__any(scr)) return F::load(bases + (size_t)(loc & ~MSM_NEG) * MsmBaseStride<G>::value);
    if (__all(scr)) return fld_ld(PT + (size_t)(loc & ~MSM_SCR) * (2 * EW * 64));
    F r = F::zero();
    if (scr) r = fld_ld(PT + (size_t)(loc & ~MSM_SCR) * (2 * EW * 64));
    else r = F::load(bases + (size_t)(loc & ~MSM_NEG) * MsmBaseStride<G>::value);
    return r; };
  auto base_point = [&](uint32_t loc) {
    Aff<F> q = Aff<F>::load(bases + (size_t)(loc & ~MSM_NEG) * MsmBaseStride<G>::value);
    const F ny = q.y.neg();
    if (loc & MSM_NEG) q.y = ny;
    return q; };
  auto scratch_point = [&](uint32_t loc) {
    const uint32_t* p = PT + (size_t)(loc & ~MSM_SCR) * (2 * EW * 64);
    Aff<F> q;
    q.x = fld_ld(p); q.y = fld_ld(p + (size_t)EW * 64);
    return q; };
  auto point_of = [&](uint32_t loc) {
    const bool scr = (loc & MSM_SCR) != 0;
    if (!__any(scr)) return base_point(loc);
    if (__all(scr)) return scratch_point(loc);
    Aff<F> q = {F::zero(), F::zero()};
    if (scr) q = scratch_point(loc);
    else q = base_point(loc);
    return q; };
  for (uint32_t w = blockIdx.x; w < nwaves; w += gridDim.x) {
    const uint32_t t = w * 64 + lane;
    const uint64_t start64 = (uint64_t)t * chunk;
    const uint32_t start = start64 < M ? (uint32_t)start64 : M;
    const uint32_t n0 = min(M - start, chunk), end = start + n0;
    uint32_t key_first = 0;
    bool open_start = false;
    if (n0) {
      MsmCursor cur;
      cur.seek(off, nkeys, start);
      key_first = cur.key;
      open_start = cur.key_start < start;
      for (uint32_t i = 0; i < n0; i++) {
        const uint32_t p = start + i;
        if (p >= cur.key_end) cur.advance_to(off, nkeys, p);
        uint32_t e;
        if (compact) e = (src.ones_idx && p >= ones_start) ? src.ones_idx[p - ones_start] : src.sorted_idx[p];
        else e = msm_entry(src, false, cur, p);
        LS[(size_t)(2 * i) * 64] = cur.key;
        LS[(size_t)(2 * i + 1) * 64] = e;
      }
    }
    uint32_t cnt = n0, which = 0, slot_base = 0;
    for (;;) {
      uint32_t* const in = LS + (size_t)which * (2 * tb.cap * 64);
      uint32_t* const out = LS + (size_t)(which ^ 1) * (2 * tb.cap * 64);
      uint32_t np = 0, j = 0;
      for (uint32_t i = 0; i < cnt; j++) {
        const uint32_t k0 = in[(size_t)(2 * i) * 64], l0 = in[(size_t)(2 * i + 1) * 64];
        if (i + 1 < cnt && in[(size_t)(2 * i + 2) * 64] == k0) {
          PR[(size_t)(3 * np) * 64] = l0;
          PR[(size_t)(3 * np + 1) * 64] = in[(size_t)(2 * i + 3) * 64];
          out[(size_t)(2 * j) * 64] = k0;
          out[(size_t)(2 * j + 1) * 64] = MSM_SCR | (slot_base + np);
          np++; i += 2;
        } else {
          out[(size_t)(2 * j) * 64] = k0;
          out[(size_t)(2 * j + 1) * 64] = l0;
          i++;
        }
      }
      const uint32_t np_max = msm_wave_max(np);
      if (np_max < min_pairs) break;
      F run = F::one();
      {
        uint32_t la = 0, lb = 0, la1 = 0, lb1 = 0;
        if (0 < np) { la = PR[0]; lb = PR[(size_t)64]; }
        if (1 < np) { la1 = PR[(size_t)3 * 64]; lb1 = PR[(size_t)4 * 64]; }
        F x1n = F::zero(), x2n = F::zero();
        if (0 < np) { x1n = x_of(la); x2n = x_of(lb); }
        for (uint32_t k = 0; k < np_max; k++) {
          const F x1 = x1n, x2 = x2n;
          const uint32_t ca = la, cb = lb;
          la = la1; lb = lb1;
          if (k + 2 < np) { la1 = PR[(size_t)(3 * k + 6) * 64]; lb1 = PR[(size_t)(3 * k + 7) * 64]; }
          if (k + 1 < np) { x1n = x_of(la); x2n = x_of(lb); }
          F dd = F::one();
          if (k < np) {
            uint32_t kind = MSM_PK_ADD;
            dd = x2 - x1;
            if (__builtin_expect(x1.is_raw_zero() || x2.is_raw_zero() || dd.is_zero(), 0)) {
              const Aff<F> a = point_of(ca), b = point_of(cb);
              if (a.is_inf()) { kind = MSM_PK_TAKE_B; dd = F::one(); }
              else if (b.is_inf()) { kind = MSM_PK_TAKE_A; dd = F::one(); }
              else if (dd.is_zero()) {
                if ((a.y + b.y).is_zero()) { kind = MSM_PK_INF; dd = F::one(); }
                else { kind = MSM_PK_DBL; dd = a.y.dbl(); }
              }
            }
            PR[(size_t)(3 * k + 2) * 64] = kind;
            fld_st(PX + (size_t)k * (EW * 64), run);
          }
          run = F::mul_impl(run, dd);
        }
      }
      F inv = run.inv_gcd();
      {
        Aff<F> an = {F::zero(), F::zero()}, bn = an;
        F pren = F::one();
        uint32_t kindn = MSM_PK_INF, la = 0, lb = 0;
        if (np_max - 1 < np) {
          const uint32_t k = np_max - 1;
          an = point_of(PR[(size_t)(3 * k) * 64]); bn = point_of(PR[(size_t)(3 * k + 1) * 64]);
          kindn = PR[(size_t)(3 * k + 2) * 64];
          pren = fld_ld(PX + (size_t)k * (EW * 64));
        }
        if (np_max >= 2 && np_max - 2 < np) { la = PR[(size_t)(3 * (np_max - 2)) * 64]; lb = PR[(size_t)(3 * (np_max - 2) + 1) * 64]; }
        for (uint32_t k = np_max; k-- > 0;) {
          const bool live = k < np;
          const uint32_t kind = live ? kindn : (uint32_t)MSM_PK_ADD;
          const F ax = an.x, ay = an.y, pre = pren;
          const F sx = an.x + bn.x;
          F dd = F::one(), num = F::zero();
          if (live && kind == MSM_PK_ADD) { dd = bn.x - an.x; num = bn.y - an.y; }
          if (__builtin_expect(__any(kind == MSM_PK_DBL), 0)) {
            if (kind == MSM_PK_DBL) { const F xx = ax.sqr(); dd = ay.dbl(); num = xx.dbl() + xx + GA::mul_by_a(F::one()); }
          }
          F t0 = F::zero(), lam = F::zero();
#pragma nounroll
          for (uint32_t ph = 0; ph < tb.phases; ph++) {
            F u, v;
            if (ph == 0) { u = inv; v = pre; }
            else if (ph == 1) { u = inv; v = dd; }
            else { u = num; v = t0; }
            const F m = F::mul_impl(u, v);
            if (ph == 0) t0 = m;
            else if (ph == 1) inv = m;
            else lam = m;
          }
          if (k >= 1 && k - 1 < np) {
            an = point_of(la); bn = point_of(lb);
            kindn = PR[(size_t)(3 * (k - 1) + 2) * 64];
            pren = fld_ld(PX + (size_t)(k - 1) * (EW * 64));
          }
          if (k >= 2 && k - 2 < np) { la = PR[(size_t)(3 * (k - 2)) * 64]; lb = PR[(size_t)(3 * (k - 2) + 1) * 64]; }
          Aff<F> r;
          r.x = F::sqr_impl(lam) - sx;
          r.y = F::mul_impl(lam, ax - r.x) - ay;
          if (__builtin_expect(__any(live && kind != MSM_PK_ADD && kind != MSM_PK_DBL), 0)) {
            if (live && kind == MSM_PK_TAKE_A) r = point_of(PR[(size_t)(3 * k) * 64]);
            if (live && kind == MSM_PK_TAKE_B) r = point_of(PR[(size_t)(3 * k + 1) * 64]);
            if (live && kind == MSM_PK_INF) r = {F::zero(), F::zero()};
          }
          if (live) {
            uint32_t* p = PT + (size_t)(slot_base + k) * (2 * EW * 64);
            fld_st(p, r.x); fld_st(p + (size_t)EW * 64, r.y);
          }
        }
      }
      slot_base += np_max;
      cnt = j;
      which ^= 1;
    }
    if (n0) {
      const uint32_t* const in = LS + (size_t)which * (2 * tb.cap * 64);
      MsmRunPlain<GA> acc;
      uint32_t key = key_first;
      for (uint32_t i = 0; i < cnt; i++) {
        const uint32_t k0 = in[(size_t)(2 * i) * 64], l0 = in[(size_t)(2 * i + 1) * 64];
        if (k0 != key) {
          if (open_start) { acc.flush(piece_first + (size_t)t * RW); open_start = false; }
          else acc.flush(buckets + (size_t)key * RW);
          key = k0;
        }
        acc.add(point_of(l0));
      }
      const bool open_end = off[key + 1] > end;
      if (open_end) acc.flush(piece_last + (size_t)t * RW);
      else if (open_start) acc.flush(piece_first + (size_t)t * RW);
      else acc.flush(buckets + (size_t)key * RW);
    }
  }
}

template <class G>
struct MsmItems {
  typedef typename SplitOfTail<G>::type GA;
  static constexpr uint32_t LANES = SplitOfTail<G>::LANES, PER_WAVE = 64 / LANES;
  PCD_DEV static bool idle() { return threadIdx.x >= PER_WAVE * LANES; }
  PCD_DEV static uint32_t local() { return threadIdx.x / LANES; }
  PCD_DEV static uint32_t item() { return blockIdx.x * PER_WAVE + threadIdx.x / LANES; }
  static uint32_t grid(uint32_t items) { return (items + PER_WAVE - 1) / PER_WAVE; }
};

static __global__ void __launch_bounds__(256) msm_zero_kernel(uint32_t* __restrict__ cnt, uint32_t n_cnt, uint32_t* __restrict__ ctl4) {
  const uint32_t i = blockIdx.x * blockDim.x + threadIdx.x;
  if (i < n_cnt) cnt[i] = 0;
  if (i < 4) ctl4[i] = 0;
}

#ifndef PCD_SINGLE_ITEM_PLAIN
#define PCD_SINGLE_ITEM_PLAIN 0
#endif
template <class G> struct MsmSingleItem {
  typedef typename std::conditional<PCD_SINGLE_ITEM_PLAIN != 0, typename SplitOf<G>::type, typename SplitOfTail<G>::type>::type GA;
  static constexpr int LANES = PCD_SINGLE_ITEM_PLAIN != 0 ? SplitOf<G>::LANES : SplitOfTail<G>::LANES;
};
template <class G>
__global__ void __launch_bounds__(64) msm_merge_ones_kernel(uint32_t* __restrict__ buckets, uint32_t ones_key) {
  typedef typename MsmSingleItem<G>::GA GA;
  typedef typename GA::F F;
  if (blockIdx.x != 0 || threadIdx.x >= MsmSingleItem<G>::LANES) return;
  Jac<F> a = Jac<F>::load(buckets + (size_t)1 * Jac<F>::WORDS);
  Jac<F> b = Jac<F>::load(buckets + (size_t)ones_key * Jac<F>::WORDS);
  EC<GA>::add(a, b).store(buckets + (size_t)1 * Jac<F>::WORDS);
}

template <class G>
__global__ void __launch_bounds__(64) msm_fixup_kernel(const uint32_t* __restrict__ off, uint32_t nkeys, const MsmChunkRule rule,
                                                       const uint32_t* __restrict__ piece_first, const uint32_t* __restrict__ piece_last,
                                                       const uint32_t* __restrict__ acc_buckets ,
                                                       uint32_t* __restrict__ buckets, uint32_t big_limit, uint32_t* __restrict__ big_count,
                                                       uint32_t* __restrict__ big_list , uint32_t big_cap,
                                                       uint32_t* __restrict__ seg_list , uint32_t seg_len) {
  const uint32_t chunk = rule.eval(off, nkeys);
  typedef typename MsmItems<G>::GA GA;
  typedef typename GA::F F;
  typedef EC<GA> E;
  constexpr int RW = MsmStored<GA>::WORDS;
  if (MsmItems<G>::idle()) return;
  const bool lead = threadIdx.x % MsmItems<G>::LANES == 0;
  const uint32_t item = MsmItems<G>::item();
  if (item < 2) {
    const uint32_t key = item == 0 ? 1u : nkeys - 1;
    const uint32_t lo = off[key], hi = off[key + 1];
    if (hi == lo) F::zero().store(buckets + (size_t)key * Jac<F>::WORDS + 2 * F::WORDS);
    else if (MsmStored<GA>::SEPARATE && hi - (lo / chunk) * chunk <= chunk)
      MsmStored<GA>::load(acc_buckets + (size_t)key * RW).store(buckets + (size_t)key * Jac<F>::WORDS);
    return;
  }
  const uint32_t t0 = item - 2;
  const uint64_t edge = ((uint64_t)t0 + 1) * chunk;
  if (edge >= off[nkeys]) return;
  const uint32_t key = msm_find_key(off, nkeys, (uint32_t)edge - 1);
  const uint32_t lo = off[key], hi = off[key + 1];
  if (hi <= (uint32_t)edge || lo / chunk != t0) return;
  const uint32_t t1 = (hi - 1) / chunk;
  if (t1 - t0 + 1 > big_limit) {
    if (!lead) return;
    uint32_t nseg = (t1 - t0 + seg_len) / seg_len;
    uint32_t slot = atomicAdd(&big_count[0], 1u);
    uint32_t s0 = atomicAdd(&big_count[1], nseg);
    if (slot < big_cap) { big_list[3 * slot] = key; big_list[3 * slot + 1] = s0; big_list[3 * slot + 2] = nseg; }
    for (uint32_t i = 0; i < nseg; i++) {
      uint32_t lo = t0 + i * seg_len, hi = min(t1, lo + seg_len - 1);
      seg_list[3 * (s0 + i)] = lo; seg_list[3 * (s0 + i) + 1] = hi; seg_list[3 * (s0 + i) + 2] = t1;
    }
    return;
  }
  Jac<F> acc = MsmStored<GA>::load(piece_last + (size_t)t0 * RW);
  for (uint32_t u = t0 + 1; u < t1; u++) acc = E::add(acc, MsmStored<GA>::load(piece_last + (size_t)u * RW));
  acc = E::add(acc, MsmStored<GA>::load(piece_first + (size_t)t1 * RW));
  acc.store(buckets + (size_t)key * Jac<F>::WORDS);
}

template <class G, bool ENABLE = true, bool Q = true>
struct MsmPairItems {
  static constexpr bool TWO = ENABLE && TwoLaneOps<G>::value && (MsmItems<G>::LANES == 1 || HalfLanes<typename MsmItems<G>::GA::F>::L == (int)MsmItems<G>::LANES);
  static constexpr bool QUAD = Q && TWO && MsmItems<G>::LANES == 1 && PCD_EC4 != 0;
  static constexpr uint32_t BASE = MsmItems<G>::LANES, LANES = QUAD ? 4 : TWO ? 2 * BASE : BASE, PER_WAVE = 64 / LANES;
  PCD_DEV static bool idle() { return threadIdx.x >= PER_WAVE * LANES; }
  PCD_DEV static uint32_t item() { return blockIdx.x * PER_WAVE + threadIdx.x / LANES; }
  PCD_DEV static uint32_t local() { return threadIdx.x / LANES; }
  PCD_DEV static bool writer() { return QUAD ? (threadIdx.x & 3u) == 0 : (!TWO || (((threadIdx.x & 63u) / BASE) & 1u) == 0); }
  static uint32_t grid(uint32_t items) { return (items + PER_WAVE - 1) / PER_WAVE; }
};
template <class G, bool TWO = MsmPairItems<G, true>::TWO, bool Q = true>
struct MsmPairOps {
  typedef typename MsmItems<G>::GA GA;
  typedef Jac<typename GA::F> J;
  PCD_DEV static J add(const J& a, const J& b) { return EC<GA>::add(a, b); }
  PCD_DEV static J dbl(const J& a) { return EC<GA>::dbl(a); }
};
template <class G, bool Q>
struct MsmPairOps<G, true, Q> {
  typedef typename SplitOfTail<G>::type GA;
  typedef Jac<typename GA::F> J;
  PCD_DEV static J add(const J& a, const J& b) { if constexpr (MsmPairItems<G, true, Q>::QUAD) return EC4<GA>::add4(a, b); else return EC2<GA>::add2(a, b); }
  PCD_DEV static J dbl(const J& a) { if constexpr (MsmPairItems<G, true, Q>::QUAD) return EC4<GA>::dbl4(a); else return EC2<GA>::dbl2(a); }
};
template <class G>
PCD_DEV void msm_wave_tree(Jac<typename MsmPairOps<G>::GA::F> acc, uint32_t* my , uint32_t* dst) {
  typedef MsmPairItems<G> IT;
  typedef MsmPairOps<G> O;
  typedef typename O::GA::F F;
  constexpr uint32_t PW = IT::PER_WAVE;
  const uint32_t it = IT::local();
  const bool live = !IT::idle();
  if (live && IT::writer()) acc.store(my + (size_t)it * Jac<F>::WORDS);
  __syncthreads();
  for (uint32_t s = 32; s > 0; s >>= 1) {
    if (live && it < s && it + s < PW) {
      Jac<F> o = Jac<F>::load(my + (size_t)(it + s) * Jac<F>::WORDS);
      acc = O::add(acc, o);
      if (IT::writer()) acc.store(my + (size_t)it * Jac<F>::WORDS);
    }
    __syncthreads();
  }
  if (live && it == 0 && IT::writer()) acc.store(dst);
  __syncthreads();
}
template <class G>
__global__ void __launch_bounds__(64) msm_big_segments_kernel(const uint32_t* __restrict__ seg_list, const uint32_t* __restrict__ big_count,
                                                              const uint32_t* __restrict__ piece_first, const uint32_t* __restrict__ piece_last,
                                                              uint32_t* __restrict__ partial, uint32_t* __restrict__ scratch) {
  typedef MsmPairItems<G> IT;
  typedef MsmPairOps<G> O;
  typedef typename O::GA GA;
  typedef typename GA::F F;
  constexpr uint32_t PW = IT::PER_WAVE;
  const uint32_t nseg = big_count[1];
  uint32_t* my = scratch + (size_t)blockIdx.x * 64 * Jac<F>::WORDS;
  for (uint32_t sg = blockIdx.x; sg < nseg; sg += gridDim.x) {
    uint32_t lo = seg_list[3 * sg], hi = seg_list[3 * sg + 1], tlast = seg_list[3 * sg + 2];
    Jac<F> acc = Jac<F>::infinity();
    if (!IT::idle())
      for (uint32_t u = lo + IT::local(); u <= hi; u += PW) {
        const uint32_t* src = (u == tlast) ? piece_first : piece_last;
        acc = O::add(acc, MsmStored<GA>::load(src + (size_t)u * MsmStored<GA>::WORDS));
      }
    msm_wave_tree<G>(acc, my, partial + (size_t)sg * Jac<F>::WORDS);
  }
}
template <class G>
__global__ void __launch_bounds__(64) msm_big_bucket_kernel(const uint32_t* __restrict__ big_list, const uint32_t* __restrict__ big_count,
                                                            const uint32_t* __restrict__ partial, uint32_t* __restrict__ buckets,
                                                            uint32_t* __restrict__ scratch) {
  typedef MsmPairItems<G> IT;
  typedef MsmPairOps<G> O;
  typedef typename O::GA GA;
  typedef typename GA::F F;
  constexpr uint32_t PW = IT::PER_WAVE;
  const uint32_t nbig = big_count[0];
  uint32_t* my = scratch + (size_t)blockIdx.x * 64 * Jac<F>::WORDS;
  for (uint32_t b = blockIdx.x; b < nbig; b += gridDim.x) {
    uint32_t key = big_list[3 * b], s0 = big_list[3 * b + 1], ns = big_list[3 * b + 2];
    Jac<F> acc = Jac<F>::infinity();
    if (!IT::idle())
      for (uint32_t u = IT::local(); u < ns; u += PW) acc = O::add(acc, Jac<F>::load(partial + (size_t)(s0 + u) * Jac<F>::WORDS));
    msm_wave_tree<G>(acc, my, buckets + (size_t)key * Jac<F>::WORDS);
  }
}

struct MsmBucketSrc {
  const uint32_t* off;
  const uint32_t* acc_buckets;
  const uint32_t* buckets;
  uint32_t nkeys;
  MsmChunkRule rule;
};
template <class GA>
PCD_DEV Jac<typename GA::F> msm_bucket_at(const MsmBucketSrc& bs, uint32_t chunk, uint32_t key) {
  typedef typename GA::F F;
  if (key != 1) {
    const uint32_t lo = bs.off[key], hi = bs.off[key + 1];
    if (hi == lo) return Jac<F>::infinity();
    if (hi - (lo / chunk) * chunk <= chunk)
      return MsmStored<GA>::load(bs.acc_buckets + (size_t)key * MsmStored<GA>::WORDS);
  }
  return Jac<F>::load(bs.buckets + (size_t)key * Jac<F>::WORDS);
}
template <class G, bool WIDE>
__global__ void __launch_bounds__(64) msm_tail_level_kernel(const MsmBucketSrc bs, uint32_t mA, size_t strideA_in,
                                                            const uint32_t* __restrict__ C_in, uint32_t mC, size_t strideC_in,
                                                            uint32_t* __restrict__ A_out, size_t strideA_out,
                                                            uint32_t* __restrict__ C_out, size_t strideC_out, int k) {
  typedef MsmPairItems<G, WIDE> IT;
  typedef MsmPairOps<G, IT::TWO> O;
  typedef typename O::GA GA;
  typedef typename GA::F F;
  constexpr int PW = Jac<F>::WORDS;
  if (IT::idle()) return;
  uint32_t K = 1u << k;
  uint32_t JA = (mA + K - 1) >> k, JC = (mC + K - 1) >> k;
  uint32_t tid = IT::item();
  uint32_t w = blockIdx.y;
  if (tid < JA) {
    const uint32_t chunk = bs.rule.eval(bs.off, bs.nkeys);
    const uint32_t key1 = w * (uint32_t)strideA_in + 1;
    Jac<F> run = Jac<F>::infinity(), acc = Jac<F>::infinity();
    for (int tt = (int)K - 1; tt >= 0; tt--) {
      uint32_t i = tid * K + tt;
      if (i < mA) run = O::add(run, msm_bucket_at<GA>(bs, chunk, key1 + i));
      acc = O::add(acc, run);
    }
    if (IT::writer()) acc.store(C_out + (w * strideC_out + JC + tid) * PW);
    if (tid >= 1) {
      for (int d = 0; d < k; d++) run = O::dbl(run);
      if (IT::writer()) run.store(A_out + (w * strideA_out + tid - 1) * PW);
    }
  } else if (tid < JA + JC) {
    uint32_t j = tid - JA;
    const uint32_t* Cw = C_in + w * strideC_in * PW;
    Jac<F> acc = Jac<F>::infinity();
    for (uint32_t tt = 0; tt < K; tt++) {
      uint32_t i = j * K + tt;
      if (i < mC) acc = O::add(acc, Jac<F>::load(Cw + (size_t)i * PW));
    }
    if (IT::writer()) acc.store(C_out + (w * strideC_out + j) * PW);
  }
}

template <class G, bool Q = true, bool FIRST = false>
PCD_DEV void msm_tail_pair_item(int role, uint32_t j, uint32_t w, const uint32_t* A_in, uint32_t mA, size_t strideA_in, const uint32_t* C_in,
                                uint32_t mC, size_t strideC_in, uint32_t* A_out, size_t strideA_out, uint32_t* C_out, size_t strideC_out,
                                const MsmBucketSrc* bs = nullptr) {
  typedef MsmPairOps<G, MsmPairItems<G, true>::TWO, Q> O;
  typedef typename O::GA GA;
  typedef typename GA::F F;
  typedef MsmPairItems<G, true, Q> IT;
  constexpr int PW = Jac<F>::WORDS;
  const uint32_t JA = (mA + 1) >> 1, JC = (mC + 1) >> 1;
  if (role < 2) {
    if (j >= JA) return;
    uint32_t chunk = 0;
    if constexpr (FIRST) chunk = bs->rule.eval(bs->off, bs->nkeys);
    auto a_at = [&](uint32_t i) {
      if constexpr (FIRST) return msm_bucket_at<GA>(*bs, chunk, w * (uint32_t)strideA_in + 1 + i);
      else return Jac<F>::load(A_in + (w * strideA_in + i) * PW);
    };
    const bool two = 2 * j + 1 < mA;
    const Jac<F> a0 = a_at(2 * j);
    if (role == 0) {
      if (j == 0) return;
      Jac<F> run = two ? O::add(a0, a_at(2 * j + 1)) : a0;
      run = O::dbl(run);
      if (IT::writer()) run.store(A_out + (w * strideA_out + j - 1) * PW);
    } else {
      Jac<F> acc = two ? O::add(O::dbl(a_at(2 * j + 1)), a0) : a0;
      if (IT::writer()) acc.store(C_out + (w * strideC_out + JC + j) * PW);
    }
  } else {
    if (j >= JC) return;
    const uint32_t* Cw = C_in + w * strideC_in * PW;
    Jac<F> acc = Jac<F>::load(Cw + (size_t)(2 * j) * PW);
    if (2 * j + 1 < mC) acc = O::add(acc, Jac<F>::load(Cw + (size_t)(2 * j + 1) * PW));
    if (IT::writer()) acc.store(C_out + (w * strideC_out + j) * PW);
  }
}
template <class G, bool Q = true>
__global__ void __launch_bounds__(64) msm_tail_pair_kernel(const uint32_t* __restrict__ A_in, uint32_t mA, size_t strideA_in,
                                                           const uint32_t* __restrict__ C_in, uint32_t mC, size_t strideC_in,
                                                           uint32_t* __restrict__ A_out, size_t strideA_out,
                                                           uint32_t* __restrict__ C_out, size_t strideC_out) {
  typedef MsmPairItems<G, true, Q> IT;
  if (IT::idle()) return;
  msm_tail_pair_item<G, Q>((int)blockIdx.z, IT::item(), blockIdx.y, A_in, mA, strideA_in, C_in, mC, strideC_in, A_out, strideA_out, C_out, strideC_out);
}
template <class G, bool Q = true>
__global__ void __launch_bounds__(64) msm_tail_pair_first_kernel(const MsmBucketSrc bs, uint32_t mA, size_t strideA_in,
                                                                 uint32_t* __restrict__ A_out, size_t strideA_out,
                                                                 uint32_t* __restrict__ C_out, size_t strideC_out) {
  typedef MsmPairItems<G, true, Q> IT;
  if (IT::idle()) return;
  msm_tail_pair_item<G, Q, true>((int)blockIdx.z, IT::item(), blockIdx.y, nullptr, mA, strideA_in, nullptr, 0u, 0, A_out, strideA_out, C_out, strideC_out, &bs);
}
constexpr uint32_t MSM_FUSED_WAVES = 4;
#ifndef PCD_QUAD_MAX_ITEMS
#define PCD_QUAD_MAX_ITEMS 4096
#endif
constexpr uint32_t MSM_QUAD_MAX_ITEMS = PCD_QUAD_MAX_ITEMS;
template <class G>
struct MsmFusedTail {
  static constexpr bool ENABLED = !MsmPairOps<G>::GA::F::Base::MAILBOX;
  static uint32_t waves(uint32_t items) { return (items + MsmPairItems<G>::PER_WAVE - 1) / MsmPairItems<G>::PER_WAVE; }
  static bool fits(uint32_t mA, uint32_t mC) { return ENABLED && 2 * waves((mA + 1) >> 1) + waves((mC + 1) >> 1) <= MSM_FUSED_WAVES; }
};
template <class G>
__global__ void __launch_bounds__(64 * MSM_FUSED_WAVES) msm_tail_fused_kernel(const uint32_t* A_in, uint32_t mA, size_t strideA_in, const uint32_t* C_in,
                                                                              uint32_t mC, size_t strideC_in, uint32_t* A0, uint32_t* A1, uint32_t* C0,
                                                                              uint32_t* C1, size_t strideAC, int flip) {
  typedef MsmPairItems<G> IT;
  const uint32_t wave = threadIdx.x >> 6, lane = threadIdx.x & 63u;
  const bool idle = lane >= IT::PER_WAVE * IT::LANES;
  const uint32_t w = blockIdx.x;
  while (mA > 0 || mC > 1) {
    const uint32_t JA = (mA + 1) >> 1, JC = (mC + 1) >> 1;
    uint32_t* A_out = flip ? A1 : A0;
    uint32_t* C_out = flip ? C1 : C0;
    const uint32_t wa = (JA + IT::PER_WAVE - 1) / IT::PER_WAVE;
    const int role = wave < wa ? 0 : wave < 2 * wa ? 1 : 2;
    const uint32_t j = (wave - (uint32_t)role * wa) * IT::PER_WAVE + lane / IT::LANES;
    if (!idle) msm_tail_pair_item<G>(role, j, w, A_in, mA, strideA_in, C_in, mC, strideC_in, A_out, strideAC, C_out, strideAC);
    __syncthreads();
    mA = JA ? JA - 1 : 0;
    mC = JC + JA;
    A_in = A_out; strideA_in = strideAC;
    C_in = C_out; strideC_in = strideAC;
    flip ^= 1;
  }
}

template <class G>
__global__ void __launch_bounds__(64) msm_horner_kernel(const uint32_t* __restrict__ C, size_t strideC, int W, int c, uint32_t* __restrict__ out) {
  typedef typename MsmSingleItem<G>::GA GA;
  typedef typename GA::F F;
  typedef EC<GA> E;
  constexpr int PW = Jac<F>::WORDS;
  if (blockIdx.x != 0 || threadIdx.x >= MsmSingleItem<G>::LANES) return;
  Jac<F> total = Jac<F>::load(C + (size_t)(W - 1) * strideC * PW);
  for (int w = W - 2; w >= 0; w--) {
    for (int d = 0; d < c; d++) total = E::dbl(total);
    total = E::add(total, Jac<F>::load(C + (size_t)w * strideC * PW));
  }
  total.store(out);
}

template <class G>
__global__ void __launch_bounds__(64) points_abi_to_internal_kernel(const uint32_t* __restrict__ abi, uint32_t n, uint32_t* __restrict__ out) {
  typedef typename G::F F;
  uint32_t i = blockIdx.x * blockDim.x + threadIdx.x;
  if (i >= n) return;
  Aff<F>::from_abi(abi + (size_t)i * Aff<F>::ABI_WORDS).store(out + (size_t)i * MsmBaseStride<G>::value);
}
template <class G>
__global__ void __launch_bounds__(64) jac_internal_to_abi_kernel(const uint32_t* __restrict__ in, uint32_t n, uint32_t* __restrict__ abi) {
  typedef typename G::F F;
  uint32_t i = blockIdx.x * blockDim.x + threadIdx.x;
  if (i >= n) return;
  Jac<F> p = Jac<F>::load(in + (size_t)i * Jac<F>::WORDS);
  if (p.is_inf()) p = Jac<F>::infinity();
  p.to_abi(abi + (size_t)i * Jac<F>::ABI_WORDS);
}

template <class G>
__global__ void __launch_bounds__(64) msm_precompute_kernel(uint32_t* __restrict__ pts, uint32_t n, int groups, int shift) {
  typedef typename std::conditional<AccOf<G>::LANES == 1, typename AccOf<G>::type, G>::type GP;
  typedef typename GP::F F;
  typedef EC<GP> E;
  constexpr int BLK = (F::Base::N > 11 || F::DEG > 1) ? 4 : 8;
  uint32_t i = blockIdx.x * blockDim.x + threadIdx.x;
  if (i >= n) return;
  constexpr int STRIDE = MsmBaseStride<G>::value;
  Aff<F> p = Aff<F>::load(pts + (size_t)i * STRIDE);
  if (p.is_inf()) {
    for (int g = 1; g < groups; g++) p.store(pts + ((size_t)g * n + i) * STRIDE);
    return;
  }
  Jac<F> q = {p.x, p.y, F::one()};
  for (int g0 = 1; g0 < groups; g0 += BLK) {
    const int nb = min(BLK, groups - g0);
    F zs[BLK], pre[BLK];
    unsigned infm = 0;
#pragma unroll
    for (int j = 0; j < BLK; j++) {
      if (j < nb) {
        for (int d = 0; d < shift; d++) q = E::dbl(q);
        uint32_t* dst = pts + ((size_t)(g0 + j) * n + i) * STRIDE;
        q.X.store(dst);
        q.Y.store(dst + F::WORDS);
        const bool inf = q.is_inf();
        if (inf) infm |= 1u << j;
        zs[j] = inf ? F::one() : q.Z;
        pre[j] = j ? pre[j - 1] * zs[j] : zs[j];
      }
    }
    F inv = pre[0];
#pragma unroll
    for (int j = 1; j < BLK; j++) if (j == nb - 1) inv = pre[j];
    inv = inv.inv();
    Aff<F> last = {F::zero(), F::zero()};
#pragma unroll
    for (int j = BLK - 1; j >= 0; j--) {
      if (j < nb) {
        const F zi = j ? inv * pre[j - 1] : inv;
        inv = inv * zs[j];
        uint32_t* dst = pts + ((size_t)(g0 + j) * n + i) * STRIDE;
        const F zi2 = zi.sqr();
        Aff<F> a = {F::load(dst) * zi2, F::load(dst + F::WORDS) * zi2 * zi};
        if (infm & (1u << j)) a = {F::zero(), F::zero()};
        a.store(dst);
        if (j == nb - 1) last = a;
      }
    }
    q = (infm >> (nb - 1)) & 1u ? Jac<F>::infinity() : Jac<F>{last.x, last.y, F::one()};
  }
}
template <class G>
hipError_t msm_precompute(hipStream_t st, uint32_t* pts, uint32_t n, int groups, int shift) {
  if (n == 0 || groups <= 1) return hipSuccess;
  hipLaunchKernelGGL((msm_precompute_kernel<G>), dim3((n + 63) / 64), dim3(64), 0, st, pts, n, groups, shift);
  return hipGetLastError();
}

struct MsmLane {
  hipStream_t stream = nullptr;
  int cus = 0;
};

struct MsmWorkspace {
  void* buf[28] = {nullptr};
  size_t cap[28] = {0};
  const MsmLane* lane = nullptr;
  hipEvent_t lane_in = nullptr, lane_out = nullptr;
  const uint32_t* last_err_dev = nullptr;
  int cus = 0;
  int bin_stage = -1;
  hipError_t ensure(int slot, size_t bytes) {
    if (cap[slot] >= bytes) return hipSuccess;
    if (buf[slot]) { hipError_t e = hipFree(buf[slot]); if (e != hipSuccess) return e; buf[slot] = nullptr; cap[slot] = 0; }
    size_t want = bytes + bytes / 8 + 256;
    hipError_t e = hipMalloc(&buf[slot], want);
    if (e != hipSuccess) return e;
    cap[slot] = want;
    return hipSuccess;
  }
  void release() {
    for (int i = 0; i < 28; i++) if (buf[i]) { (void)hipFree(buf[i]); buf[i] = nullptr; cap[i] = 0; }
    if (lane_in) { (void)hipEventDestroy(lane_in); lane_in = nullptr; }
    if (lane_out) { (void)hipEventDestroy(lane_out); lane_out = nullptr; }
  }
};

struct MsmTimings {
  float digits = 0, scan = 0, scatter = 0, accumulate = 0, fixup = 0, tail = 0, horner = 0, total = 0;
  uint32_t entries = 0, chunk = 0;
};

enum { WS_CNT = 0, WS_OFF, WS_BSUM, WS_SORTED, WS_BUCKETS, WS_PFIRST, WS_PLAST, WS_BIG, WS_BIGSCR, WS_A0, WS_A1, WS_C0, WS_C1, WS_OUT, WS_SCAL,
       WS_BIGPART, WS_ONES, WS_SLOTS, WS_CUR, WS_ENTRIES, WS_ACCB, WS_TLIST, WS_TPAIR, WS_TPREFIX, WS_TPTS };

#define PCD_HIP_TRY(x) do { hipError_t e_ = (x); if (e_ != hipSuccess) return e_; } while (0)

struct MsmBasesView {
  const uint32_t* dptr;
  uint32_t n_total;
  uint32_t offset;
  int c;
  int groups;
  const uint32_t* inf_bits = nullptr;
};

struct MsmSharedSort {
  bool valid = false;
  uint32_t n = 0, n_total = 0, offset = 0, tkeys = 0;
  int c = 0, W = 0, groups = 0;
  const uint32_t* scalars = nullptr;
  const uint32_t* inf_bits = nullptr;
  MsmEntrySource src{};
  const uint32_t* off = nullptr;
  hipEvent_t ready = nullptr;
};
enum { MSM_SHARE_NONE = 0, MSM_SHARE_PRODUCE = 1, MSM_SHARE_CONSUME = 2 };

template <class G>
hipError_t msm_run(MsmWorkspace& ws, hipStream_t st, const MsmBasesView& bv, const uint32_t* scalars_dev, uint32_t n,
                   uint32_t* out_dev, int c_override, uint32_t chunk_override, int sort_mode, MsmTimings* tm,
                   MsmSharedSort* share = nullptr, int share_role = MSM_SHARE_NONE) {
  const int acc_mode = (sort_mode >> 4) & 3;
  const uint32_t tree_chunk = ((uint32_t)sort_mode >> 8) & 0xFFFu, tree_min_pairs = ((uint32_t)sort_mode >> 20) & 0xFFu;
  sort_mode &= 15;
  const bool single_pass = sort_mode == 1;
  const uint32_t* bases_dev = bv.dptr;
  typedef typename G::F F;
  constexpr int NS = G::FR::N32;
  constexpr int PW = Jac<F>::WORDS;
  constexpr size_t PB = (size_t)PW * 4;
  if (n == 0) { ws.last_err_dev = nullptr; Jac<F> inf = Jac<F>::infinity(); return hipMemcpyAsync(out_dev, &inf, PB, hipMemcpyHostToDevice, st); }
  MsmPlan pl;
  pl.n = n;
  pl.c = bv.groups > 1 ? bv.c : (c_override ? c_override : msm_pick_window(n, G::FR::BITS, 0));
  pl.W = msm_num_windows(G::FR::BITS, pl.c);
  const int Wg = (pl.W + bv.groups - 1) / bv.groups;
  pl.nkeys = (uint32_t)Wg << pl.c;
  const uint64_t maxM = (uint64_t)n * pl.W;
  pl.chunk = chunk_override ? chunk_override : 40;
  int& cus = ws.cus;
  if (!cus) {
    int dev = 0;
    if (hipGetDevice(&dev) != hipSuccess || hipDeviceGetAttribute(&cus, hipDeviceAttributeMultiprocessorCount, dev) != hipSuccess || cus <= 0) cus = 256;
  }
  bool use_tree = false;
  uint32_t tree_cap = 0;
  const uint32_t* tree_chunk_dev = nullptr;
  if constexpr (MsmTreeCapable<G>::value) {
    use_tree = acc_mode == 2 && (uint64_t)bv.n_total * bv.groups < MSM_SCR;
    if (use_tree) {
      tree_cap = tree_chunk ? tree_chunk : MSM_TREE_CHUNK_MAX;
      pl.chunk = tree_cap;
    }
  }
  const MsmLane* lane = ws.lane;
  const int plan_cus = lane && lane->cus > 0 ? lane->cus : cus;
  uint32_t acc_lanes = 0, chunk_lo = 0;
  static const uint32_t chunk_hi_env = getenv("PCDHIP_CHUNK_HI") ? (uint32_t)atoi(getenv("PCDHIP_CHUNK_HI")) : 0u;
  const uint32_t chunk_hi = chunk_hi_env >= 16 && chunk_hi_env <= MSM_CHUNK_MAX ? chunk_hi_env : MSM_CHUNK_HI;
  if (!chunk_override && !use_tree) {
    acc_lanes = (uint32_t)plan_cus * 4 * MsmAccWaves<G>::value * (64 / AccOf<G>::LANES);
    chunk_lo = (uint32_t)std::min<uint64_t>(40, std::max<uint64_t>(16, (maxM + 4ull * acc_lanes - 1) / (4ull * acc_lanes)));
    pl.chunk = chunk_lo;
  }
  const uint64_t plan_word = acc_lanes && acc_lanes < (1u << 20) ? msm_plan_word(acc_lanes, chunk_lo, chunk_hi) : 0u;
  if (acc_lanes && !plan_word) pl.chunk = 40;
  if (maxM >= 0xFFFFFFF0ull || (uint64_t)bv.n_total * bv.groups >= 0x7FFFFFF0ull) return hipErrorInvalidValue;

  EventSet<9> ev;
  if (tm) PCD_HIP_TRY(ev.create());
  auto mark = [&](int i) -> hipError_t { return tm ? hipEventRecord(ev[i], st) : hipSuccess; };

  const uint32_t tkeys = pl.nkeys + 1, ones_key = pl.nkeys;
  const bool consume = share && share_role == MSM_SHARE_CONSUME && share->valid && share->n == n && share->n_total == bv.n_total &&
                       share->offset == bv.offset && share->tkeys == tkeys && share->c == pl.c && share->W == pl.W &&
                       share->groups == bv.groups && share->scalars == scalars_dev &&
                       (share->inf_bits == nullptr || share->inf_bits == bv.inf_bits);
  PCD_HIP_TRY(ws.ensure(WS_CNT, (size_t)tkeys * 4 + 16));
  PCD_HIP_TRY(ws.ensure(WS_OFF, ((size_t)tkeys + 1) * 4));
  const uint32_t scan_per_block = 16384;
  const uint32_t scan_blocks = (tkeys + scan_per_block - 1) / scan_per_block;
  PCD_HIP_TRY(ws.ensure(WS_BSUM, (size_t)scan_blocks * 4));
  PCD_HIP_TRY(ws.ensure(WS_SORTED, (size_t)maxM * 4));
  PCD_HIP_TRY(ws.ensure(WS_BUCKETS, (size_t)tkeys * PB));
  PCD_HIP_TRY(ws.ensure(WS_OUT, PB + 64));
  PCD_HIP_TRY(ws.ensure(WS_ONES, (size_t)n * 4 + 32));
  uint32_t* cnt = (uint32_t*)ws.buf[WS_CNT];
  uint32_t* off = (uint32_t*)ws.buf[WS_OFF];
  uint32_t* bsum = (uint32_t*)ws.buf[WS_BSUM];
  uint32_t* sorted = (uint32_t*)ws.buf[WS_SORTED];
  uint32_t* buckets = (uint32_t*)ws.buf[WS_BUCKETS];
  uint32_t* ones_idx = (uint32_t*)ws.buf[WS_ONES];
  uint32_t* flag = ones_idx + n;
  uint32_t* err = flag + 1;
  uint32_t* big_count = flag + 2;
  auto zero_start = [&](uint32_t n_cnt) {
    hipLaunchKernelGGL(msm_zero_kernel, dim3(std::max<uint32_t>(1u, (n_cnt + 255) / 256)), dim3(256), 0, st, cnt, n_cnt, flag);
  };
  ws.last_err_dev = consume ? nullptr : err;
  constexpr int SBITS = G::FR::BITS;
  const int wins = (pl.W + Wg - 1) / Wg;
  const int top_bits = G::FR::BITS + 1 - (pl.W - 1) * pl.c;
  double mu = (double)n * wins / (double)(1u << (pl.c - 1)) + (top_bits < pl.c ? (double)n / (double)(1u << top_bits) : 0.0);
  uint32_t cap = (uint32_t)(mu + 6.0 * sqrt(mu) + 8.0);
  cap = (cap + 7u) & ~7u;
  const bool use_slots = single_pass && (double)pl.nkeys * cap * 4.0 <= 1.5e9;
  const uint32_t nbins = pl.nkeys >> MSM_BIN_SHIFT;
  const bool use_partition = (sort_mode == 0 || sort_mode == 3 || sort_mode == 4) && pl.c >= MSM_BIN_SHIFT && nbins >= 1 && nbins <= MSM_MAX_BINS && n >= 4096;
  uint32_t stage_tile = 0;
  if (use_partition && sort_mode != 3) {
    const int knob = msm_coarse_tile_knob();
    stage_tile = knob == 0 ? 0u : msm_stage_tile(pl.W, nbins);
    while (knob > 0 && stage_tile > (uint32_t)knob) stage_tile >>= 1;
  }
  const uint32_t bin_cap = sort_mode == 4 || msm_bin_stage_knob() == 0 ? 0u
                           : ws.bin_stage < 0 ? MSM_BIN_STAGE_CAP : std::min<uint32_t>((uint32_t)ws.bin_stage, MSM_BIN_STAGE_CAP);
  uint32_t* slots = nullptr;
  if (use_slots) { PCD_HIP_TRY(ws.ensure(WS_SLOTS, (size_t)pl.nkeys * cap * 4)); slots = (uint32_t*)ws.buf[WS_SLOTS]; }

  PCD_HIP_TRY(mark(0));
  dim3 gd((n + 255) / 256), bd(256);
  MsmEntrySource src;
  if (consume) {
    PCD_HIP_TRY(hipStreamWaitEvent(st, share->ready, 0));
    zero_start(0);
    src = share->src;
    off = const_cast<uint32_t*>(share->off);
    PCD_HIP_TRY(mark(1)); PCD_HIP_TRY(mark(2)); PCD_HIP_TRY(mark(3));
  } else if (use_slots) {
    zero_start(tkeys);
    hipLaunchKernelGGL((msm_digits_kernel<NS, MODE_BIN>), gd, bd, 0, st, scalars_dev, n, pl.c, pl.W, Wg, bv.n_total, bv.offset, pl.nkeys, cnt,
                       (const uint32_t*)nullptr, (uint32_t*)nullptr, slots, cap, ones_idx, flag, 0, SBITS, err, bv.inf_bits);
    PCD_HIP_TRY(mark(1));
    hipLaunchKernelGGL(scan_block_sums, dim3(scan_blocks), dim3(1024), 0, st, cnt, tkeys, scan_per_block, bsum);
    hipLaunchKernelGGL(scan_apply, dim3(scan_blocks), dim3(1024), 0, st, cnt, tkeys, scan_per_block, bsum, scan_blocks, off);
    PCD_HIP_TRY(mark(2));
    PCD_HIP_TRY(ws.ensure(WS_CUR, (size_t)tkeys * 4));
    uint32_t* cur = (uint32_t*)ws.buf[WS_CUR];
    PCD_HIP_TRY(hipMemsetAsync(cur, 0, (size_t)tkeys * 4, st));
    hipLaunchKernelGGL((msm_digits_kernel<NS, MODE_SCATTER>), gd, bd, 0, st, scalars_dev, n, pl.c, pl.W, Wg, bv.n_total, bv.offset, pl.nkeys, cur,
                       off, sorted, (uint32_t*)nullptr, 0u, (uint32_t*)nullptr, flag, 1, SBITS, err, bv.inf_bits);
    PCD_HIP_TRY(mark(3));
    src = {sorted, slots, ones_idx, flag, cap, ones_key};
  } else if (use_partition) {
    zero_start(nbins + 1);
    const uint32_t tiles = (n + MSM_TILE - 1) / MSM_TILE;
    PCD_HIP_TRY(ws.ensure(WS_ENTRIES, (size_t)maxM * 8));
    PCD_HIP_TRY(ws.ensure(WS_CUR, ((size_t)2 * nbins + 8) * 4));
    uint64_t* entries = (uint64_t*)ws.buf[WS_ENTRIES];
    uint32_t* bin_base = (uint32_t*)ws.buf[WS_CUR];
    uint32_t* cursor = bin_base + nbins + 2;
    uint32_t* ones_count = flag;
    hipLaunchKernelGGL((msm_coarse_kernel<NS, false>), dim3(tiles), dim3(256), (size_t)nbins * 4, st, scalars_dev, n, pl.c, pl.W, Wg, bv.n_total,
                       bv.offset, nbins, cnt, (uint64_t*)nullptr, ones_count, ones_idx, SBITS, err, bv.inf_bits);
    PCD_HIP_TRY(mark(1));
    hipLaunchKernelGGL(msm_bin_scan_kernel, dim3(1), dim3(1024), 0, st, cnt, nbins, bin_base, cursor, ones_count, off, pl.nkeys);
    PCD_HIP_TRY(mark(2));
    if (stage_tile) {
      const uint32_t stiles = (n + stage_tile - 1) / stage_tile;
      const size_t lds = msm_stage_lds_bytes(stage_tile, pl.W, nbins);
#define PCD_STAGED(T) msm_coarse_staged_launch<NS, T>(st, stiles, lds, scalars_dev, n, pl.c, pl.W, Wg, bv.n_total, bv.offset, nbins, cursor, entries, bv.inf_bits)
      PCD_HIP_TRY(stage_tile == 2048 ? PCD_STAGED(2048) : stage_tile == 1024 ? PCD_STAGED(1024) : stage_tile == 512 ? PCD_STAGED(512) : PCD_STAGED(256));
#undef PCD_STAGED
    } else {
      hipLaunchKernelGGL((msm_coarse_kernel<NS, true>), dim3(tiles), dim3(256), (size_t)nbins * 4, st, scalars_dev, n, pl.c, pl.W, Wg, bv.n_total,
                         bv.offset, nbins, cursor, entries, ones_count, ones_idx, SBITS, err, bv.inf_bits);
    }
    PCD_HIP_TRY(msm_bin_sort_launch(st, nbins, bin_cap, entries, bin_base, sorted, off));
    PCD_HIP_TRY(mark(3));
    src = {sorted, nullptr, ones_idx, nullptr, 0u, ones_key};
  } else {
    zero_start(tkeys);
    hipLaunchKernelGGL((msm_digits_kernel<NS, MODE_HIST>), gd, bd, 0, st, scalars_dev, n, pl.c, pl.W, Wg, bv.n_total, bv.offset, pl.nkeys, cnt,
                       (const uint32_t*)nullptr, (uint32_t*)nullptr, (uint32_t*)nullptr, 0u, (uint32_t*)nullptr, (uint32_t*)nullptr, 0, SBITS, err, bv.inf_bits);
    PCD_HIP_TRY(mark(1));
    hipLaunchKernelGGL(scan_block_sums, dim3(scan_blocks), dim3(1024), 0, st, cnt, tkeys, scan_per_block, bsum);
    hipLaunchKernelGGL(scan_apply, dim3(scan_blocks), dim3(1024), 0, st, cnt, tkeys, scan_per_block, bsum, scan_blocks, off);
    PCD_HIP_TRY(mark(2));
    PCD_HIP_TRY(hipMemsetAsync(cnt, 0, (size_t)tkeys * 4, st));
    hipLaunchKernelGGL((msm_digits_kernel<NS, MODE_SCATTER>), gd, bd, 0, st, scalars_dev, n, pl.c, pl.W, Wg, bv.n_total, bv.offset, pl.nkeys, cnt,
                       off, sorted, (uint32_t*)nullptr, 0u, (uint32_t*)nullptr, (uint32_t*)nullptr, 0, SBITS, err, bv.inf_bits);
    PCD_HIP_TRY(mark(3));
    src = {sorted, nullptr, nullptr, nullptr, 0u, ones_key};
  }
  if (share && share_role == MSM_SHARE_PRODUCE) {
    share->valid = true;
    share->n = n; share->n_total = bv.n_total; share->offset = bv.offset; share->tkeys = tkeys;
    share->c = pl.c; share->W = pl.W; share->groups = bv.groups; share->scalars = scalars_dev; share->inf_bits = bv.inf_bits;
    share->src = src; share->off = off;
    PCD_HIP_TRY(hipEventRecord(share->ready, st));
  }
  uint32_t nchunks = (uint32_t)((maxM + pl.chunk - 1) / pl.chunk);
  uint32_t tree_grid = 0;
  if (use_tree) {
    tree_grid = std::min<uint32_t>(tree_chunk ? (nchunks + 63) / 64 : (uint32_t)((maxM / 32 + 63) / 64), (uint32_t)plan_cus * 4);
    if (!tree_chunk) nchunks = tree_grid * 64 * (uint32_t)((maxM + (uint64_t)tree_grid * 64 * tree_cap - 1) / ((uint64_t)tree_grid * 64 * tree_cap));
  }
  typedef MsmStored<typename SplitOf<G>::type> Stored;
  constexpr size_t RB = (size_t)Stored::WORDS * 4;
  PCD_HIP_TRY(ws.ensure(WS_PFIRST, (size_t)nchunks * RB));
  PCD_HIP_TRY(ws.ensure(WS_PLAST, (size_t)nchunks * RB));
  uint32_t* acc_buckets = buckets;
  if (Stored::SEPARATE) { PCD_HIP_TRY(ws.ensure(WS_ACCB, (size_t)tkeys * RB)); acc_buckets = (uint32_t*)ws.buf[WS_ACCB]; }
  const uint32_t big_limit = 8, seg_len = 128;
  const uint32_t big_cap = nchunks / big_limit + 2;
  const uint32_t seg_cap = nchunks / seg_len + big_cap + 2;
  PCD_HIP_TRY(ws.ensure(WS_BIG, (size_t)(3 * big_cap + 3 * seg_cap + 8) * 4));
  PCD_HIP_TRY(ws.ensure(WS_BIGPART, (size_t)seg_cap * PB));
  uint32_t* pfirst = (uint32_t*)ws.buf[WS_PFIRST];
  uint32_t* plast = (uint32_t*)ws.buf[WS_PLAST];
  uint32_t* big = (uint32_t*)ws.buf[WS_BIG];
  uint32_t* seg_list = big + 3 * big_cap;
  uint32_t* big_partial = (uint32_t*)ws.buf[WS_BIGPART];
  PCD_HIP_TRY(mark(8));
  hipStream_t own = st;
  if (lane) {
    if (!ws.lane_in) PCD_HIP_TRY(hipEventCreateWithFlags(&ws.lane_in, hipEventDisableTiming));
    if (!ws.lane_out) PCD_HIP_TRY(hipEventCreateWithFlags(&ws.lane_out, hipEventDisableTiming));
    PCD_HIP_TRY(hipEventRecord(ws.lane_in, own));
    PCD_HIP_TRY(hipStreamWaitEvent(lane->stream, ws.lane_in, 0));
    st = lane->stream;
  }
  {
    constexpr uint32_t per_wave = 64 / AccOf<G>::LANES;
    const dim3 acc_grid((nchunks + per_wave - 1) / per_wave);
    bool launched = false;
    if constexpr (MsmTreeCapable<G>::value) {
      if (use_tree) {
        constexpr int FW = AccOf<G>::type::F::WORDS;
        const uint32_t grid = tree_grid;
        MsmTreeBufs tb;
        tb.cap = tree_cap;
        tb.phases = 3;
        uint32_t* chunk_word = big_count + 2;
        hipLaunchKernelGGL(msm_tree_plan_kernel, dim3(1), dim3(1), 0, st, off, tkeys, grid * 64, tree_cap, tree_chunk, chunk_word);
        tree_chunk_dev = chunk_word;
        PCD_HIP_TRY(ws.ensure(WS_TLIST, MsmTreeBufs::list_words(tb.cap) * 4 * grid));
        PCD_HIP_TRY(ws.ensure(WS_TPAIR, MsmTreeBufs::pair_words(tb.cap) * 4 * grid));
        PCD_HIP_TRY(ws.ensure(WS_TPREFIX, MsmTreeBufs::prefix_words(tb.cap, FW) * 4 * grid));
        PCD_HIP_TRY(ws.ensure(WS_TPTS, MsmTreeBufs::pts_words(tb.cap, FW) * 4 * grid));
        tb.list = (uint32_t*)ws.buf[WS_TLIST]; tb.pairs = (uint32_t*)ws.buf[WS_TPAIR];
        tb.prefix = (uint32_t*)ws.buf[WS_TPREFIX]; tb.pts = (uint32_t*)ws.buf[WS_TPTS];
        hipLaunchKernelGGL((msm_pair_tree_kernel<G>), dim3(grid), dim3(64), 0, st, bases_dev, src, off, tkeys, chunk_word, tb,
                           tree_min_pairs ? tree_min_pairs : MSM_TREE_MIN_PAIRS, acc_buckets, pfirst, plast);
        launched = true;
      }
    }
    if (!launched) {
      if (src.slots) hipLaunchKernelGGL((msm_accumulate_kernel<G, false>), acc_grid, dim3(64), 0, st, bases_dev, src, off, tkeys, pl.chunk, acc_buckets, pfirst, plast, plan_word);
      hipLaunchKernelGGL((msm_accumulate_kernel<G, true>), acc_grid, dim3(64), 0, st, bases_dev, src, off, tkeys, pl.chunk, acc_buckets, pfirst, plast, plan_word);
    }
  }
  if (lane) {
    PCD_HIP_TRY(hipEventRecord(ws.lane_out, st));
    st = own;
    PCD_HIP_TRY(hipStreamWaitEvent(st, ws.lane_out, 0));
  }
  PCD_HIP_TRY(mark(4));
  const MsmChunkRule chunk_rule = {tree_chunk_dev, plan_word, pl.chunk};
  hipLaunchKernelGGL((msm_fixup_kernel<G>), dim3(MsmItems<G>::grid(nchunks + 2)), dim3(64), 0, st, off, tkeys, chunk_rule, pfirst, plast, acc_buckets,
                     buckets, big_limit, big_count, big, big_cap, seg_list, seg_len);
  {
    const uint32_t big_grid = std::min<uint32_t>(seg_cap, 2048);
    PCD_HIP_TRY(ws.ensure(WS_BIGSCR, (size_t)big_grid * 64 * PB));
    hipLaunchKernelGGL((msm_big_segments_kernel<G>), dim3(big_grid), dim3(64), 0, st, seg_list, big_count, pfirst, plast, big_partial,
                       (uint32_t*)ws.buf[WS_BIGSCR]);
    hipLaunchKernelGGL((msm_big_bucket_kernel<G>), dim3(std::min<uint32_t>(big_cap, 2048)), dim3(64), 0, st, big, big_count, big_partial,
                       buckets, (uint32_t*)ws.buf[WS_BIGSCR]);
  }
  hipLaunchKernelGGL((msm_merge_ones_kernel<G>), dim3(1), dim3(64), 0, st, buckets, ones_key);
  PCD_HIP_TRY(mark(5));
  {
    const uint32_t B = 1u << (pl.c - 1);
    size_t cap_pts = ((size_t)1 << pl.c);
    PCD_HIP_TRY(ws.ensure(WS_A0, (size_t)Wg * cap_pts * PB / 2 + PB * Wg * 4));
    PCD_HIP_TRY(ws.ensure(WS_A1, (size_t)Wg * cap_pts * PB / 2 + PB * Wg * 4));
    PCD_HIP_TRY(ws.ensure(WS_C0, (size_t)Wg * cap_pts * PB / 2 + PB * Wg * 4));
    PCD_HIP_TRY(ws.ensure(WS_C1, (size_t)Wg * cap_pts * PB / 2 + PB * Wg * 4));
    const size_t strideAC = cap_pts / 2 + 4;
    const MsmBucketSrc bucket_src = {off, acc_buckets, buckets, tkeys, chunk_rule};
    const uint32_t* A_in = buckets + PW;
    size_t strideA_in = (size_t)1 << pl.c;
    const uint32_t* C_in = nullptr;
    size_t strideC_in = 0;
    uint32_t mA = B, mC = 0;
    int flip = 0, level = 0;
    bool fused = false;
    while (mA > 0 || mC > 1) {
      int k = (level == 0 && B >= (1u << 17)) ? 3 : 1;
      uint32_t K = 1u << k;
      uint32_t JA = (mA + K - 1) >> k, JC = (mC + K - 1) >> k;
      uint32_t* A_out = (uint32_t*)ws.buf[flip ? WS_A1 : WS_A0];
      uint32_t* C_out = (uint32_t*)ws.buf[flip ? WS_C1 : WS_C0];
      uint32_t threads = JA + JC;
      if (!fused && level > 0 && MsmFusedTail<G>::fits(mA, mC)) {
        hipLaunchKernelGGL((msm_tail_fused_kernel<G>), dim3(Wg), dim3(64 * MSM_FUSED_WAVES), 0, st, A_in, mA, strideA_in, C_in, mC, strideC_in,
                           (uint32_t*)ws.buf[WS_A0], (uint32_t*)ws.buf[WS_A1], (uint32_t*)ws.buf[WS_C0], (uint32_t*)ws.buf[WS_C1], strideAC, flip);
        fused = true;
      }
      if (fused) {
      } else if (level == 0 && k == 1 && JA * (uint32_t)Wg > MSM_QUAD_MAX_ITEMS)
        hipLaunchKernelGGL((msm_tail_pair_first_kernel<G, false>), dim3(MsmPairItems<G, true, false>::grid(JA), Wg, 2), dim3(64), 0, st, bucket_src, mA,
                           strideA_in, A_out, strideAC, C_out, strideAC);
      else if (level == 0 && k == 1)
        hipLaunchKernelGGL((msm_tail_pair_first_kernel<G>), dim3(MsmPairItems<G>::grid(JA), Wg, 2), dim3(64), 0, st, bucket_src, mA, strideA_in, A_out,
                           strideAC, C_out, strideAC);
      else if (k == 1 && std::max(JA, JC) * (uint32_t)Wg > MSM_QUAD_MAX_ITEMS)
        hipLaunchKernelGGL((msm_tail_pair_kernel<G, false>), dim3(MsmPairItems<G, true, false>::grid(std::max(JA, JC)), Wg, 3), dim3(64), 0, st, A_in, mA,
                           strideA_in, C_in, mC, strideC_in, A_out, strideAC, C_out, strideAC);
      else if (k == 1)
        hipLaunchKernelGGL((msm_tail_pair_kernel<G>), dim3(MsmPairItems<G>::grid(std::max(JA, JC)), Wg, 3), dim3(64), 0, st, A_in, mA, strideA_in, C_in,
                           mC, strideC_in, A_out, strideAC, C_out, strideAC);
      else if (threads <= (1u << 15))
        hipLaunchKernelGGL((msm_tail_level_kernel<G, true>), dim3(MsmPairItems<G, true>::grid(threads), Wg), dim3(64), 0, st, bucket_src, mA, strideA_in, C_in,
                           mC, strideC_in, A_out, strideAC, C_out, strideAC, k);
      else
        hipLaunchKernelGGL((msm_tail_level_kernel<G, false>), dim3(MsmPairItems<G, false>::grid(threads), Wg), dim3(64), 0, st, bucket_src, mA, strideA_in, C_in,
                           mC, strideC_in, A_out, strideAC, C_out, strideAC, k);
      mA = JA ? JA - 1 : 0;
      mC = JC + JA;
      A_in = A_out; strideA_in = strideAC;
      C_in = C_out; strideC_in = strideAC;
      flip ^= 1;
      level++;
    }
    PCD_HIP_TRY(mark(6));
    hipLaunchKernelGGL((msm_horner_kernel<G>), dim3(1), dim3(64), 0, st, C_in, strideC_in, Wg, pl.c, out_dev);
    PCD_HIP_TRY(mark(7));
  }
  PCD_HIP_TRY(hipGetLastError());
  if (tm) {
    PCD_HIP_TRY(hipStreamSynchronize(st));
    auto el = [&](int a, int b) { float ms = 0; (void)hipEventElapsedTime(&ms, ev[a], ev[b]); return ms; };
    tm->digits = el(0, 1); tm->scan = el(1, 2); tm->scatter = el(2, 8); tm->accumulate = el(8, 4);
    tm->fixup = el(4, 5); tm->tail = el(5, 6); tm->horner = el(6, 7); tm->total = el(0, 7);
    PCD_HIP_TRY(hipMemcpy(&tm->entries, off + tkeys, 4, hipMemcpyDeviceToHost));
    tm->chunk = plan_word ? msm_chunk_of_plan(tm->entries, plan_word) : pl.chunk;
    if (tree_chunk_dev) PCD_HIP_TRY(hipMemcpy(&tm->chunk, tree_chunk_dev, 4, hipMemcpyDeviceToHost));
  }
  return hipSuccess;
}

}
```

Measured before the change: 422.3 Mscalar-mul/s.

## Fuse MSM output conversion into horner, cache edge keys, drop merge-ones kernel

Several changes at once. The horner kernel now writes the ABI-format result and error flag directly, so the separate jac_out launch and the second error readback go away, and a single copy into pinned host memory replaces them. The accumulate kernel records each chunk's starting key so the fixup kernel can skip its binary search. The ones-bucket merge kernel is replaced by a pseudo item injected into the first tail level. The tail level schedule is also restructured into a rule/step helper with an optional fan-3 reduction. These changes mainly cut launch count and small-transfer latency, at the cost of extra control-flow complexity and a new workspace buffer.

Result: no change. 421.7 Mscalar-mul/s (-0.1%).

```diff
diff --git a/pcd_amd/csrc/capi_internal.h b/pcd_amd/csrc/capi_internal.h
--- a/pcd_amd/csrc/capi_internal.h
+++ b/pcd_amd/csrc/capi_internal.h
@@ -58,6 +58,7 @@
 int bases_upload_single(pcdhip_ctx* ctx, int curve_id, int group_id, const uint64_t* xy, const uint8_t* inf, size_t n, pcdhip_bases** out);
 int msm_common(pcdhip_ctx* ctx, const pcdhip_bases* bases, size_t offset, const uint32_t* scalars_dev, size_t n, uint64_t* out_xyz,
                bool out_on_device = false);
+int ensure_pipe_host(pcdhip_ctx* ctx);
 int ensure_side_streams(pcdhip_ctx* ctx);
 int drop_side_streams(pcdhip_ctx* ctx, bool partial);
 bool pipe_pending(const pcdhip_ctx* ctx);
diff --git a/pcd_amd/csrc/capi_msm.hip b/pcd_amd/csrc/capi_msm.hip
--- a/pcd_amd/csrc/capi_msm.hip
+++ b/pcd_amd/csrc/capi_msm.hip
@@ -153,15 +153,26 @@
   TRY(ctx->msm_ws.ensure(WS_OUT, jac_b + jac_abi_b + 64));
   uint32_t* out_dev = (uint32_t*)ctx->msm_ws.buf[WS_OUT];
   uint32_t* out_abi = out_dev + jac_b / 4;
-  TRY(ge.msm(ctx->msm_ws, ctx->stream, bases->view(offset), scalars_dev, (uint32_t)n, out_dev, ctx->msm_c, ctx->msm_chunk,
-             ctx->msm_sort, ctx->msm_profile ? &ctx->msm_tm : nullptr, nullptr, MSM_SHARE_NONE));
+  if (!out_on_device) { const int rc = ensure_pipe_host(ctx); if (rc) return rc; }
+  ctx->msm_ws.abi_out = out_on_device ? nullptr : out_abi;
+  const hipError_t me = ge.msm(ctx->msm_ws, ctx->stream, bases->view(offset), scalars_dev, (uint32_t)n, out_dev, ctx->msm_c, ctx->msm_chunk,
+                               ctx->msm_sort, ctx->msm_profile ? &ctx->msm_tm : nullptr, nullptr, MSM_SHARE_NONE);
+  ctx->msm_ws.abi_out = nullptr;
+  TRY(me);
   if (out_on_device) { TRY(ge.jac_out(ctx->stream, out_dev, 1, (uint32_t*)out_xyz)); return PCDHIP_OK; }
-  TRY(ge.jac_out(ctx->stream, out_dev, 1, out_abi));
-  TRY(hipMemcpyAsync(out_xyz, out_abi, jac_abi_b, hipMemcpyDeviceToHost, ctx->stream));
+  uint64_t* host = ctx->pipe_host + (size_t)pcdhip_ctx::PIPE_SLOTS * pcdhip_ctx::PIPE_HOST_WORDS;
+  TRY(hipMemcpyAsync(host, out_abi, jac_abi_b + 4, hipMemcpyDeviceToHost, ctx->stream));
+  TRY(hipStreamSynchronize(ctx->stream));
+  memcpy(out_xyz, host, jac_abi_b);
   uint32_t too_wide = 0;
-  if (ctx->msm_ws.last_err_dev) TRY(hipMemcpyAsync(&too_wide, ctx->msm_ws.last_err_dev, 4, hipMemcpyDeviceToHost, ctx->stream));
-  TRY(hipStreamSynchronize(ctx->stream));
+  memcpy(&too_wide, (const char*)host + jac_abi_b, 4);
   return too_wide ? PCDHIP_E_ARG : PCDHIP_OK;
+}
+
+int ensure_pipe_host(pcdhip_ctx* ctx) {
+  if (!ctx->pipe_host)
+    TRY(hipHostMalloc((void**)&ctx->pipe_host, (pcdhip_ctx::PIPE_SLOTS + 1) * pcdhip_ctx::PIPE_HOST_WORDS * 8, hipHostMallocDefault));
+  return PCDHIP_OK;
 }
 
 int ensure_side_streams(pcdhip_ctx* ctx) {
@@ -213,7 +224,8 @@
   }
   if (slot < 0) return PCDHIP_E_ARG;
   ctx->pipe_next = (slot + 1) % pcdhip_ctx::PIPE_SLOTS;
-  if (!ctx->pipe_host) TRY(hipHostMalloc((void**)&ctx->pipe_host, pcdhip_ctx::PIPE_SLOTS * pcdhip_ctx::PIPE_HOST_WORDS * 8, hipHostMallocDefault));
+  rc = ensure_pipe_host(ctx);
+  if (rc) return rc;
   if (!ctx->pipe_done[slot]) TRY(hipEventCreateWithFlags(&ctx->pipe_done[slot], hipEventDisableTiming));
   bool prev_bad = false;
   if (ctx->pipe_partial[slot]) {
@@ -232,15 +244,20 @@
   TRY(hipStreamWaitEvent(sk, ctx->g16_ready, 0));
   const size_t sw = (size_t)kFieldLimbs[scalars->field_id] * 2;
   ws.lane = ctx->g16_schedule == 2 && ctx->pipe_lane && ctx->lane.stream ? &ctx->lane : nullptr;
+  ws.abi_out = out_xyz_device ? nullptr : out_abi;
   const hipError_t me = ge.msm(ws, sk, bases->view(offset), scalars->dptr + scalar_offset * sw, (uint32_t)n, out_dev, ctx->msm_c, ctx->msm_chunk, ctx->msm_sort,
                                nullptr, nullptr, MSM_SHARE_NONE);
   ws.lane = nullptr;
+  ws.abi_out = nullptr;
   TRY(me);
-  TRY(ge.jac_out(sk, out_dev, 1, out_abi));
   uint64_t* host = ctx->pipe_host + (size_t)slot * pcdhip_ctx::PIPE_HOST_WORDS;
   host[pcdhip_ctx::PIPE_HOST_WORDS - 1] = 0;
-  if (!out_xyz_device) TRY(hipMemcpyAsync(host, out_abi, jac_abi_b, hipMemcpyDeviceToHost, sk));
-  if (ws.last_err_dev) TRY(hipMemcpyAsync(&host[pcdhip_ctx::PIPE_HOST_WORDS - 1], ws.last_err_dev, 4, hipMemcpyDeviceToHost, sk));
+  if (!out_xyz_device) {
+    TRY(hipMemcpyAsync(host, out_abi, jac_abi_b + 4, hipMemcpyDeviceToHost, sk));
+  } else {
+    TRY(ge.jac_out(sk, out_dev, 1, out_abi));
+    if (ws.last_err_dev) TRY(hipMemcpyAsync(&host[pcdhip_ctx::PIPE_HOST_WORDS - 1], ws.last_err_dev, 4, hipMemcpyDeviceToHost, sk));
+  }
   TRY(hipEventRecord(ctx->pipe_done[slot], sk));
   ctx->pipe_busy[slot] = true;
   ctx->pipe_out_bytes[slot] = out_xyz_device ? 0 : jac_abi_b;
@@ -468,7 +485,9 @@
   TRY(hipEventSynchronize(ctx->pipe_done[ticket]));
   const uint64_t* host = ctx->pipe_host + (size_t)ticket * pcdhip_ctx::PIPE_HOST_WORDS;
   memcpy(out_xyz, host, ctx->pipe_out_bytes[ticket]);
-  return (uint32_t)host[pcdhip_ctx::PIPE_HOST_WORDS - 1] ? PCDHIP_E_ARG : PCDHIP_OK;
+  uint32_t too_wide = 0;
+  memcpy(&too_wide, (const char*)host + ctx->pipe_out_bytes[ticket], 4);
+  return too_wide ? PCDHIP_E_ARG : PCDHIP_OK;
 }
 
 int pcdhip_msm_dev(pcdhip_ctx* ctx, const pcdhip_bases* bases, size_t offset, const pcdhip_buf* scalars, size_t scalar_offset,
diff --git a/pcd_amd/csrc/msm.hip.h b/pcd_amd/csrc/msm.hip.h
--- a/pcd_amd/csrc/msm.hip.h
+++ b/pcd_amd/csrc/msm.hip.h
@@ -768,6 +768,7 @@
                                                             const uint32_t* __restrict__ off, uint32_t nkeys,
                                                             uint32_t chunk, uint32_t* __restrict__ buckets,
                                                             uint32_t* __restrict__ piece_first, uint32_t* __restrict__ piece_last,
+                                                            uint32_t* __restrict__ edge_key ,
                                                             uint64_t plan ) {
   if (plan) chunk = msm_chunk_of_plan(off[nkeys], plan);
   typedef typename AccOf<G>::type GA;
@@ -785,6 +786,7 @@
   if (COMPACT && src.flag && *src.flag == 0) return;
   MsmCursor cur;
   cur.seek(off, nkeys, start);
+  edge_key[t] = cur.key;
   bool open_start = cur.key_start < start;
 #if PCD_ACC_LDS
   typename std::conditional<LazyCapable<F>::value, MsmRunLazyLds<GA>, MsmRunPlain<GA>>::type acc;
@@ -1123,18 +1125,10 @@
   typedef typename std::conditional<PCD_SINGLE_ITEM_PLAIN != 0, typename SplitOf<G>::type, typename SplitOfTail<G>::type>::type GA;
   static constexpr int LANES = PCD_SINGLE_ITEM_PLAIN != 0 ? SplitOf<G>::LANES : SplitOfTail<G>::LANES;
 };
-template <class G>
-__global__ void __launch_bounds__(64) msm_merge_ones_kernel(uint32_t* __restrict__ buckets, uint32_t ones_key) {
-  typedef typename MsmSingleItem<G>::GA GA;
-  typedef typename GA::F F;
-  if (blockIdx.x != 0 || threadIdx.x >= MsmSingleItem<G>::LANES) return;
-  Jac<F> a = Jac<F>::load(buckets + (size_t)1 * Jac<F>::WORDS);
-  Jac<F> b = Jac<F>::load(buckets + (size_t)ones_key * Jac<F>::WORDS);
-  EC<GA>::add(a, b).store(buckets + (size_t)1 * Jac<F>::WORDS);
-}
 
 template <class G>
 __global__ void __launch_bounds__(64) msm_fixup_kernel(const uint32_t* __restrict__ off, uint32_t nkeys, const MsmChunkRule rule,
+                                                       const uint32_t* __restrict__ edge_key ,
                                                        const uint32_t* __restrict__ piece_first, const uint32_t* __restrict__ piece_last,
                                                        const uint32_t* __restrict__ acc_buckets ,
                                                        uint32_t* __restrict__ buckets, uint32_t big_limit, uint32_t* __restrict__ big_count,
@@ -1159,9 +1153,9 @@
   const uint32_t t0 = item - 2;
   const uint64_t edge = ((uint64_t)t0 + 1) * chunk;
   if (edge >= off[nkeys]) return;
-  const uint32_t key = msm_find_key(off, nkeys, (uint32_t)edge - 1);
+  const uint32_t key = edge_key ? edge_key[t0 + 1] : msm_find_key(off, nkeys, (uint32_t)edge - 1);
   const uint32_t lo = off[key], hi = off[key + 1];
-  if (hi <= (uint32_t)edge || lo / chunk != t0) return;
+  if (lo >= (uint32_t)edge || hi <= (uint32_t)edge || lo / chunk != t0) return;
   const uint32_t t1 = (hi - 1) / chunk;
   if (t1 - t0 + 1 > big_limit) {
     if (!lead) return;
@@ -1287,11 +1281,16 @@
   }
   return Jac<F>::load(bs.buckets + (size_t)key * Jac<F>::WORDS);
 }
+template <class GA>
+PCD_DEV Jac<typename GA::F> msm_pseudo_item(const MsmBucketSrc& bs, uint32_t w) {
+  typedef typename GA::F F;
+  return w == 0 ? Jac<F>::load(bs.buckets + (size_t)(bs.nkeys - 1) * Jac<F>::WORDS) : Jac<F>::infinity();
+}
 template <class G, bool WIDE>
 __global__ void __launch_bounds__(64) msm_tail_level_kernel(const MsmBucketSrc bs, uint32_t mA, size_t strideA_in,
                                                             const uint32_t* __restrict__ C_in, uint32_t mC, size_t strideC_in,
                                                             uint32_t* __restrict__ A_out, size_t strideA_out,
-                                                            uint32_t* __restrict__ C_out, size_t strideC_out, int k) {
+                                                            uint32_t* __restrict__ C_out, size_t strideC_out, int k, bool pseudo) {
   typedef MsmPairItems<G, WIDE> IT;
   typedef MsmPairOps<G, IT::TWO> O;
   typedef typename O::GA GA;
@@ -1325,19 +1324,73 @@
       if (i < mC) acc = O::add(acc, Jac<F>::load(Cw + (size_t)i * PW));
     }
     if (IT::writer()) acc.store(C_out + (w * strideC_out + j) * PW);
-  }
+  } else if (pseudo && tid == JA + JC) {
+    const Jac<F> p = msm_pseudo_item<GA>(bs, w);
+    if (IT::writer()) p.store(C_out + (w * strideC_out + JC + JA) * PW);
+  }
+}
+
+constexpr uint32_t MSM_FUSED_WAVES = 4;
+#ifndef PCD_QUAD_MAX_ITEMS
+#define PCD_QUAD_MAX_ITEMS 4096
+#endif
+constexpr uint32_t MSM_QUAD_MAX_ITEMS = PCD_QUAD_MAX_ITEMS;
+#ifndef PCD_BAG_FAN3
+#define PCD_BAG_FAN3 0
+#endif
+enum MsmTailKind { MSM_TAIL_FIRST8 = 0, MSM_TAIL_FIRST_PAIR, MSM_TAIL_PAIR2, MSM_TAIL_PAIR4, MSM_TAIL_FUSED };
+struct MsmTailRule {
+  uint32_t B, Wg;
+  uint32_t per_wave;
+  bool quad;
+  bool fused;
+  bool pseudo;
+};
+struct MsmTailStep {
+  uint32_t mA, mC;
+  uint32_t JA, JC;
+  uint32_t fan;
+  int k, kind;
+};
+PCD_HD constexpr size_t msm_tail_stride(uint32_t B) { return (size_t)B + 4; }
+PCD_HD uint32_t msm_tail_waves(const MsmTailRule& r, uint32_t items) { return (items + r.per_wave - 1) / r.per_wave; }
+PCD_HD bool msm_tail_fused_fits(const MsmTailRule& r, uint32_t mA, uint32_t mC, uint32_t fan) {
+  return r.fused && 2 * msm_tail_waves(r, (mA + 1) >> 1) + msm_tail_waves(r, (mC + fan - 1) / fan) <= MSM_FUSED_WAVES;
+}
+PCD_HD MsmTailStep msm_tail_step(const MsmTailRule& r, uint32_t mA, uint32_t mC, int level, bool in_fused) {
+  MsmTailStep s;
+  s.k = (level == 0 && r.B >= (1u << 17)) ? 3 : 1;
+  s.JA = (mA + (1u << s.k) - 1) >> s.k;
+  s.fan = 2;
+  const uint32_t fan_late = r.quad && PCD_BAG_FAN3 != 0 ? 3u : 2u;
+  if (level == 0) s.kind = s.k == 3 ? MSM_TAIL_FIRST8 : MSM_TAIL_FIRST_PAIR;
+  else if (in_fused || msm_tail_fused_fits(r, mA, mC, fan_late)) { s.kind = MSM_TAIL_FUSED; s.fan = fan_late; }
+  else if ((s.JA > ((mC + 1) >> 1) ? s.JA : (mC + 1) >> 1) * r.Wg > MSM_QUAD_MAX_ITEMS) s.kind = MSM_TAIL_PAIR2;
+  else { s.kind = MSM_TAIL_PAIR4; s.fan = fan_late; }
+  s.JC = (mC + s.fan - 1) / s.fan;
+  s.mA = s.JA ? s.JA - 1 : 0;
+  s.mC = s.JC + s.JA + (level == 0 && r.pseudo ? 1u : 0u);
+  return s;
+}
+template <class G>
+struct MsmFusedTail {
+  static constexpr bool ENABLED = !MsmPairOps<G>::GA::F::Base::MAILBOX;
+};
+template <class G>
+MsmTailRule msm_tail_rule(uint32_t B, uint32_t Wg, bool pseudo) {
+  return {B, Wg, MsmPairItems<G>::PER_WAVE, MsmPairItems<G>::QUAD, MsmFusedTail<G>::ENABLED, pseudo};
 }
 
 template <class G, bool Q = true, bool FIRST = false>
 PCD_DEV void msm_tail_pair_item(int role, uint32_t j, uint32_t w, const uint32_t* A_in, uint32_t mA, size_t strideA_in, const uint32_t* C_in,
                                 uint32_t mC, size_t strideC_in, uint32_t* A_out, size_t strideA_out, uint32_t* C_out, size_t strideC_out,
-                                const MsmBucketSrc* bs = nullptr) {
+                                uint32_t fan , const MsmBucketSrc* bs = nullptr) {
   typedef MsmPairOps<G, MsmPairItems<G, true>::TWO, Q> O;
   typedef typename O::GA GA;
   typedef typename GA::F F;
   typedef MsmPairItems<G, true, Q> IT;
   constexpr int PW = Jac<F>::WORDS;
-  const uint32_t JA = (mA + 1) >> 1, JC = (mC + 1) >> 1;
+  const uint32_t JA = (mA + 1) >> 1, JC = (mC + fan - 1) / fan;
   if (role < 2) {
     if (j >= JA) return;
     uint32_t chunk = 0;
@@ -1360,8 +1413,10 @@
   } else {
     if (j >= JC) return;
     const uint32_t* Cw = C_in + w * strideC_in * PW;
-    Jac<F> acc = Jac<F>::load(Cw + (size_t)(2 * j) * PW);
-    if (2 * j + 1 < mC) acc = O::add(acc, Jac<F>::load(Cw + (size_t)(2 * j + 1) * PW));
+    const uint32_t i0 = fan * j;
+    Jac<F> acc = Jac<F>::load(Cw + (size_t)i0 * PW);
+    if (i0 + 1 < mC) acc = O::add(acc, Jac<F>::load(Cw + (size_t)(i0 + 1) * PW));
+    if (PCD_BAG_FAN3 != 0 && fan == 3 && i0 + 2 < mC) acc = O::add(acc, Jac<F>::load(Cw + (size_t)(i0 + 2) * PW));
     if (IT::writer()) acc.store(C_out + (w * strideC_out + j) * PW);
   }
 }
@@ -1369,57 +1424,56 @@
 __global__ void __launch_bounds__(64) msm_tail_pair_kernel(const uint32_t* __restrict__ A_in, uint32_t mA, size_t strideA_in,
                                                            const uint32_t* __restrict__ C_in, uint32_t mC, size_t strideC_in,
                                                            uint32_t* __restrict__ A_out, size_t strideA_out,
-                                                           uint32_t* __restrict__ C_out, size_t strideC_out) {
+                                                           uint32_t* __restrict__ C_out, size_t strideC_out, uint32_t fan) {
   typedef MsmPairItems<G, true, Q> IT;
   if (IT::idle()) return;
-  msm_tail_pair_item<G, Q>((int)blockIdx.z, IT::item(), blockIdx.y, A_in, mA, strideA_in, C_in, mC, strideC_in, A_out, strideA_out, C_out, strideC_out);
+  msm_tail_pair_item<G, Q>((int)blockIdx.z, IT::item(), blockIdx.y, A_in, mA, strideA_in, C_in, mC, strideC_in, A_out, strideA_out, C_out, strideC_out, fan);
 }
 template <class G, bool Q = true>
 __global__ void __launch_bounds__(64) msm_tail_pair_first_kernel(const MsmBucketSrc bs, uint32_t mA, size_t strideA_in,
                                                                  uint32_t* __restrict__ A_out, size_t strideA_out,
-                                                                 uint32_t* __restrict__ C_out, size_t strideC_out) {
+                                                                 uint32_t* __restrict__ C_out, size_t strideC_out, bool pseudo) {
   typedef MsmPairItems<G, true, Q> IT;
   if (IT::idle()) return;
-  msm_tail_pair_item<G, Q, true>((int)blockIdx.z, IT::item(), blockIdx.y, nullptr, mA, strideA_in, nullptr, 0u, 0, A_out, strideA_out, C_out, strideC_out, &bs);
-}
-constexpr uint32_t MSM_FUSED_WAVES = 4;
-#ifndef PCD_QUAD_MAX_ITEMS
-#define PCD_QUAD_MAX_ITEMS 4096
-#endif
-constexpr uint32_t MSM_QUAD_MAX_ITEMS = PCD_QUAD_MAX_ITEMS;
-template <class G>
-struct MsmFusedTail {
-  static constexpr bool ENABLED = !MsmPairOps<G>::GA::F::Base::MAILBOX;
-  static uint32_t waves(uint32_t items) { return (items + MsmPairItems<G>::PER_WAVE - 1) / MsmPairItems<G>::PER_WAVE; }
-  static bool fits(uint32_t mA, uint32_t mC) { return ENABLED && 2 * waves((mA + 1) >> 1) + waves((mC + 1) >> 1) <= MSM_FUSED_WAVES; }
-};
-template <class G>
-__global__ void __launch_bounds__(64 * MSM_FUSED_WAVES) msm_tail_fused_kernel(const uint32_t* A_in, uint32_t mA, size_t strideA_in, const uint32_t* C_in,
-                                                                              uint32_t mC, size_t strideC_in, uint32_t* A0, uint32_t* A1, uint32_t* C0,
-                                                                              uint32_t* C1, size_t strideAC, int flip) {
+  const uint32_t JA = (mA + 1) >> 1;
+  if (pseudo && blockIdx.z == 1 && IT::item() == JA) {
+    typedef typename MsmPairOps<G, MsmPairItems<G, true>::TWO, Q>::GA GA;
+    const Jac<typename GA::F> p = msm_pseudo_item<GA>(bs, blockIdx.y);
+    if (IT::writer()) p.store(C_out + (blockIdx.y * strideC_out + JA) * Jac<typename GA::F>::WORDS);
+    return;
+  }
+  msm_tail_pair_item<G, Q, true>((int)blockIdx.z, IT::item(), blockIdx.y, nullptr, mA, strideA_in, nullptr, 0u, 0, A_out, strideA_out, C_out, strideC_out, 2u, &bs);
+}
+template <class G>
+__global__ void __launch_bounds__(64 * MSM_FUSED_WAVES) msm_tail_fused_kernel(const MsmTailRule rule, int level, const uint32_t* A_in, uint32_t mA,
+                                                                              size_t strideA_in, const uint32_t* C_in, uint32_t mC, size_t strideC_in,
+                                                                              uint32_t* A0, uint32_t* A1, uint32_t* C0, uint32_t* C1, size_t strideAC,
+                                                                              int flip) {
   typedef MsmPairItems<G> IT;
   const uint32_t wave = threadIdx.x >> 6, lane = threadIdx.x & 63u;
   const bool idle = lane >= IT::PER_WAVE * IT::LANES;
   const uint32_t w = blockIdx.x;
   while (mA > 0 || mC > 1) {
-    const uint32_t JA = (mA + 1) >> 1, JC = (mC + 1) >> 1;
+    const MsmTailStep s = msm_tail_step(rule, mA, mC, level, true);
     uint32_t* A_out = flip ? A1 : A0;
     uint32_t* C_out = flip ? C1 : C0;
-    const uint32_t wa = (JA + IT::PER_WAVE - 1) / IT::PER_WAVE;
+    const uint32_t wa = (s.JA + IT::PER_WAVE - 1) / IT::PER_WAVE;
     const int role = wave < wa ? 0 : wave < 2 * wa ? 1 : 2;
     const uint32_t j = (wave - (uint32_t)role * wa) * IT::PER_WAVE + lane / IT::LANES;
-    if (!idle) msm_tail_pair_item<G>(role, j, w, A_in, mA, strideA_in, C_in, mC, strideC_in, A_out, strideAC, C_out, strideAC);
+    if (!idle) msm_tail_pair_item<G>(role, j, w, A_in, mA, strideA_in, C_in, mC, strideC_in, A_out, strideAC, C_out, strideAC, s.fan);
     __syncthreads();
-    mA = JA ? JA - 1 : 0;
-    mC = JC + JA;
+    mA = s.mA;
+    mC = s.mC;
     A_in = A_out; strideA_in = strideAC;
     C_in = C_out; strideC_in = strideAC;
     flip ^= 1;
-  }
-}
-
-template <class G>
-__global__ void __launch_bounds__(64) msm_horner_kernel(const uint32_t* __restrict__ C, size_t strideC, int W, int c, uint32_t* __restrict__ out) {
+    level++;
+  }
+}
+
+template <class G>
+__global__ void __launch_bounds__(64) msm_horner_kernel(const uint32_t* __restrict__ C, size_t strideC, int W, int c, uint32_t* __restrict__ out,
+                                                        uint32_t* __restrict__ abi_out, const uint32_t* __restrict__ err_word) {
   typedef typename MsmSingleItem<G>::GA GA;
   typedef typename GA::F F;
   typedef EC<GA> E;
@@ -1431,6 +1485,11 @@
     total = E::add(total, Jac<F>::load(C + (size_t)w * strideC * PW));
   }
   total.store(out);
+  if (abi_out) {
+    if (total.is_inf()) total = Jac<F>::infinity();
+    total.to_abi(abi_out);
+    if (threadIdx.x == 0) abi_out[Jac<typename G::F>::ABI_WORDS] = err_word ? *err_word : 0u;
+  }
 }
 
 template <class G>
@@ -1520,6 +1579,7 @@
   size_t cap[28] = {0};
   const MsmLane* lane = nullptr;
   hipEvent_t lane_in = nullptr, lane_out = nullptr;
+  uint32_t* abi_out = nullptr;
   const uint32_t* last_err_dev = nullptr;
   int cus = 0;
   int bin_stage = -1;
@@ -1545,7 +1605,7 @@
 };
 
 enum { WS_CNT = 0, WS_OFF, WS_BSUM, WS_SORTED, WS_BUCKETS, WS_PFIRST, WS_PLAST, WS_BIG, WS_BIGSCR, WS_A0, WS_A1, WS_C0, WS_C1, WS_OUT, WS_SCAL,
-       WS_BIGPART, WS_ONES, WS_SLOTS, WS_CUR, WS_ENTRIES, WS_ACCB, WS_TLIST, WS_TPAIR, WS_TPREFIX, WS_TPTS };
+       WS_BIGPART, WS_ONES, WS_SLOTS, WS_CUR, WS_ENTRIES, WS_ACCB, WS_TLIST, WS_TPAIR, WS_TPREFIX, WS_TPTS, WS_EDGEKEY };
 
 #define PCD_HIP_TRY(x) do { hipError_t e_ = (x); if (e_ != hipSuccess) return e_; } while (0)
 
@@ -1583,7 +1643,17 @@
   constexpr int NS = G::FR::N32;
   constexpr int PW = Jac<F>::WORDS;
   constexpr size_t PB = (size_t)PW * 4;
-  if (n == 0) { ws.last_err_dev = nullptr; Jac<F> inf = Jac<F>::infinity(); return hipMemcpyAsync(out_dev, &inf, PB, hipMemcpyHostToDevice, st); }
+  if (n == 0) {
+    ws.last_err_dev = nullptr;
+    Jac<F> inf = Jac<F>::infinity();
+    if (ws.abi_out) {
+      uint32_t rec[Jac<F>::ABI_WORDS + 1];
+      inf.to_abi(rec);
+      rec[Jac<F>::ABI_WORDS] = 0;
+      PCD_HIP_TRY(hipMemcpyAsync(ws.abi_out, rec, sizeof rec, hipMemcpyHostToDevice, st));
+    }
+    return hipMemcpyAsync(out_dev, &inf, PB, hipMemcpyHostToDevice, st);
+  }
   MsmPlan pl;
   pl.n = n;
   pl.c = bv.groups > 1 ? bv.c : (c_override ? c_override : msm_pick_window(n, G::FR::BITS, 0));
@@ -1761,8 +1831,10 @@
   const uint32_t seg_cap = nchunks / seg_len + big_cap + 2;
   PCD_HIP_TRY(ws.ensure(WS_BIG, (size_t)(3 * big_cap + 3 * seg_cap + 8) * 4));
   PCD_HIP_TRY(ws.ensure(WS_BIGPART, (size_t)seg_cap * PB));
+  PCD_HIP_TRY(ws.ensure(WS_EDGEKEY, (size_t)nchunks * 4));
   uint32_t* pfirst = (uint32_t*)ws.buf[WS_PFIRST];
   uint32_t* plast = (uint32_t*)ws.buf[WS_PLAST];
+  uint32_t* edge_key = (uint32_t*)ws.buf[WS_EDGEKEY];
   uint32_t* big = (uint32_t*)ws.buf[WS_BIG];
   uint32_t* seg_list = big + 3 * big_cap;
   uint32_t* big_partial = (uint32_t*)ws.buf[WS_BIGPART];
@@ -1801,8 +1873,8 @@
       }
     }
     if (!launched) {
-      if (src.slots) hipLaunchKernelGGL((msm_accumulate_kernel<G, false>), acc_grid, dim3(64), 0, st, bases_dev, src, off, tkeys, pl.chunk, acc_buckets, pfirst, plast, plan_word);
-      hipLaunchKernelGGL((msm_accumulate_kernel<G, true>), acc_grid, dim3(64), 0, st, bases_dev, src, off, tkeys, pl.chunk, acc_buckets, pfirst, plast, plan_word);
+      if (src.slots) hipLaunchKernelGGL((msm_accumulate_kernel<G, false>), acc_grid, dim3(64), 0, st, bases_dev, src, off, tkeys, pl.chunk, acc_buckets, pfirst, plast, edge_key, plan_word);
+      hipLaunchKernelGGL((msm_accumulate_kernel<G, true>), acc_grid, dim3(64), 0, st, bases_dev, src, off, tkeys, pl.chunk, acc_buckets, pfirst, plast, edge_key, plan_word);
     }
   }
   if (lane) {
@@ -1812,7 +1884,8 @@
   }
   PCD_HIP_TRY(mark(4));
   const MsmChunkRule chunk_rule = {tree_chunk_dev, plan_word, pl.chunk};
-  hipLaunchKernelGGL((msm_fixup_kernel<G>), dim3(MsmItems<G>::grid(nchunks + 2)), dim3(64), 0, st, off, tkeys, chunk_rule, pfirst, plast, acc_buckets,
+  hipLaunchKernelGGL((msm_fixup_kernel<G>), dim3(MsmItems<G>::grid(nchunks + 2)), dim3(64), 0, st, off, tkeys, chunk_rule,
+                     use_tree ? (const uint32_t*)nullptr : edge_key , pfirst, plast, acc_buckets,
                      buckets, big_limit, big_count, big, big_cap, seg_list, seg_len);
   {
     const uint32_t big_grid = std::min<uint32_t>(seg_cap, 2048);
@@ -1822,7 +1895,6 @@
     hipLaunchKernelGGL((msm_big_bucket_kernel<G>), dim3(std::min<uint32_t>(big_cap, 2048)), dim3(64), 0, st, big, big_count, big_partial,
                        buckets, (uint32_t*)ws.buf[WS_BIGSCR]);
   }
-  hipLaunchKernelGGL((msm_merge_ones_kernel<G>), dim3(1), dim3(64), 0, st, buckets, ones_key);
   PCD_HIP_TRY(mark(5));
   {
     const uint32_t B = 1u << (pl.c - 1);
@@ -1831,8 +1903,9 @@
     PCD_HIP_TRY(ws.ensure(WS_A1, (size_t)Wg * cap_pts * PB / 2 + PB * Wg * 4));
     PCD_HIP_TRY(ws.ensure(WS_C0, (size_t)Wg * cap_pts * PB / 2 + PB * Wg * 4));
     PCD_HIP_TRY(ws.ensure(WS_C1, (size_t)Wg * cap_pts * PB / 2 + PB * Wg * 4));
-    const size_t strideAC = cap_pts / 2 + 4;
+    const size_t strideAC = msm_tail_stride(B);
     const MsmBucketSrc bucket_src = {off, acc_buckets, buckets, tkeys, chunk_rule};
+    const MsmTailRule rule = msm_tail_rule<G>(B, (uint32_t)Wg, true);
     const uint32_t* A_in = buckets + PW;
     size_t strideA_in = (size_t)1 << pl.c;
     const uint32_t* C_in = nullptr;
@@ -1841,45 +1914,43 @@
     int flip = 0, level = 0;
     bool fused = false;
     while (mA > 0 || mC > 1) {
-      int k = (level == 0 && B >= (1u << 17)) ? 3 : 1;
-      uint32_t K = 1u << k;
-      uint32_t JA = (mA + K - 1) >> k, JC = (mC + K - 1) >> k;
+      const MsmTailStep s = msm_tail_step(rule, mA, mC, level, fused);
+      const uint32_t JA = s.JA, JC = s.JC;
       uint32_t* A_out = (uint32_t*)ws.buf[flip ? WS_A1 : WS_A0];
       uint32_t* C_out = (uint32_t*)ws.buf[flip ? WS_C1 : WS_C0];
-      uint32_t threads = JA + JC;
-      if (!fused && level > 0 && MsmFusedTail<G>::fits(mA, mC)) {
-        hipLaunchKernelGGL((msm_tail_fused_kernel<G>), dim3(Wg), dim3(64 * MSM_FUSED_WAVES), 0, st, A_in, mA, strideA_in, C_in, mC, strideC_in,
-                           (uint32_t*)ws.buf[WS_A0], (uint32_t*)ws.buf[WS_A1], (uint32_t*)ws.buf[WS_C0], (uint32_t*)ws.buf[WS_C1], strideAC, flip);
+      if (s.kind == MSM_TAIL_FUSED) {
+        if (!fused)
+          hipLaunchKernelGGL((msm_tail_fused_kernel<G>), dim3(Wg), dim3(64 * MSM_FUSED_WAVES), 0, st, rule, level, A_in, mA, strideA_in, C_in, mC,
+                             strideC_in, (uint32_t*)ws.buf[WS_A0], (uint32_t*)ws.buf[WS_A1], (uint32_t*)ws.buf[WS_C0], (uint32_t*)ws.buf[WS_C1],
+                             strideAC, flip);
         fused = true;
-      }
-      if (fused) {
-      } else if (level == 0 && k == 1 && JA * (uint32_t)Wg > MSM_QUAD_MAX_ITEMS)
-        hipLaunchKernelGGL((msm_tail_pair_first_kernel<G, false>), dim3(MsmPairItems<G, true, false>::grid(JA), Wg, 2), dim3(64), 0, st, bucket_src, mA,
-                           strideA_in, A_out, strideAC, C_out, strideAC);
-      else if (level == 0 && k == 1)
-        hipLaunchKernelGGL((msm_tail_pair_first_kernel<G>), dim3(MsmPairItems<G>::grid(JA), Wg, 2), dim3(64), 0, st, bucket_src, mA, strideA_in, A_out,
-                           strideAC, C_out, strideAC);
-      else if (k == 1 && std::max(JA, JC) * (uint32_t)Wg > MSM_QUAD_MAX_ITEMS)
+      } else if (s.kind == MSM_TAIL_FIRST_PAIR && JA * (uint32_t)Wg > MSM_QUAD_MAX_ITEMS)
+        hipLaunchKernelGGL((msm_tail_pair_first_kernel<G, false>), dim3(MsmPairItems<G, true, false>::grid(JA + 1), Wg, 2), dim3(64), 0, st, bucket_src,
+                           mA, strideA_in, A_out, strideAC, C_out, strideAC, rule.pseudo);
+      else if (s.kind == MSM_TAIL_FIRST_PAIR)
+        hipLaunchKernelGGL((msm_tail_pair_first_kernel<G>), dim3(MsmPairItems<G>::grid(JA + 1), Wg, 2), dim3(64), 0, st, bucket_src, mA, strideA_in, A_out,
+                           strideAC, C_out, strideAC, rule.pseudo);
+      else if (s.kind == MSM_TAIL_PAIR2)
         hipLaunchKernelGGL((msm_tail_pair_kernel<G, false>), dim3(MsmPairItems<G, true, false>::grid(std::max(JA, JC)), Wg, 3), dim3(64), 0, st, A_in, mA,
-                           strideA_in, C_in, mC, strideC_in, A_out, strideAC, C_out, strideAC);
-      else if (k == 1)
+                           strideA_in, C_in, mC, strideC_in, A_out, strideAC, C_out, strideAC, s.fan);
+      else if (s.kind == MSM_TAIL_PAIR4)
         hipLaunchKernelGGL((msm_tail_pair_kernel<G>), dim3(MsmPairItems<G>::grid(std::max(JA, JC)), Wg, 3), dim3(64), 0, st, A_in, mA, strideA_in, C_in,
-                           mC, strideC_in, A_out, strideAC, C_out, strideAC);
-      else if (threads <= (1u << 15))
-        hipLaunchKernelGGL((msm_tail_level_kernel<G, true>), dim3(MsmPairItems<G, true>::grid(threads), Wg), dim3(64), 0, st, bucket_src, mA, strideA_in, C_in,
-                           mC, strideC_in, A_out, strideAC, C_out, strideAC, k);
+                           mC, strideC_in, A_out, strideAC, C_out, strideAC, s.fan);
+      else if (JA + JC <= (1u << 15))
+        hipLaunchKernelGGL((msm_tail_level_kernel<G, true>), dim3(MsmPairItems<G, true>::grid(JA + JC + 1), Wg), dim3(64), 0, st, bucket_src, mA, strideA_in,
+                           C_in, mC, strideC_in, A_out, strideAC, C_out, strideAC, s.k, rule.pseudo);
       else
-        hipLaunchKernelGGL((msm_tail_level_kernel<G, false>), dim3(MsmPairItems<G, false>::grid(threads), Wg), dim3(64), 0, st, bucket_src, mA, strideA_in, C_in,
-                           mC, strideC_in, A_out, strideAC, C_out, strideAC, k);
-      mA = JA ? JA - 1 : 0;
-      mC = JC + JA;
+        hipLaunchKernelGGL((msm_tail_level_kernel<G, false>), dim3(MsmPairItems<G, false>::grid(JA + JC + 1), Wg), dim3(64), 0, st, bucket_src, mA, strideA_in,
+                           C_in, mC, strideC_in, A_out, strideAC, C_out, strideAC, s.k, rule.pseudo);
+      mA = s.mA;
+      mC = s.mC;
       A_in = A_out; strideA_in = strideAC;
       C_in = C_out; strideC_in = strideAC;
       flip ^= 1;
       level++;
     }
     PCD_HIP_TRY(mark(6));
-    hipLaunchKernelGGL((msm_horner_kernel<G>), dim3(1), dim3(64), 0, st, C_in, strideC_in, Wg, pl.c, out_dev);
+    hipLaunchKernelGGL((msm_horner_kernel<G>), dim3(1), dim3(64), 0, st, C_in, strideC_in, Wg, pl.c, out_dev, ws.abi_out, ws.last_err_dev);
     PCD_HIP_TRY(mark(7));
   }
   PCD_HIP_TRY(hipGetLastError());
```
